# aleph-zero-foundation/sha2-on-cq-halo2

Hardware: AMD Instinct MI355X
Metric: sha256_cq_create_proof_k18: MSM Mscalar/s over proof-generation wall-clock (ms_per_step) (higher is better)
Workload: dtype u256-montgomery

## Files before the change

### sha2_on_cq_halo2_amd/csrc/curve.hpp

```cpp
#pragma once
#include "field.hpp"

namespace cq {

struct alignas(16) G1Affine {
  Fq x, y;
  CQ_HD bool is_identity() const { return x.is_zero() && y.is_zero(); }
  static CQ_HD G1Affine identity() { return {Fq::zero(), Fq::zero()}; }
  CQ_HD G1Affine neg() const { return {x, y.is_zero() ? y : y.neg()}; }
};

struct alignas(16) G1Jac {
  Fq x, y, z;
  static CQ_HD G1Jac identity() { return {Fq::zero(), Fq::zero(), Fq::zero()}; }
  CQ_HD bool is_identity() const { return z.is_zero(); }
};

struct XYZZ {
  Fq x, y, zz, zzz;
  static CQ_HD XYZZ identity() { return {Fq::zero(), Fq::zero(), Fq::zero(), Fq::zero()}; }
  CQ_HD bool is_identity() const { return zz.is_zero(); }
  static CQ_HD XYZZ from_affine(const G1Affine& a) {
    if (a.is_identity()) return identity();
    return {a.x, a.y, Fq::one(), Fq::one()};
  }
  CQ_HD G1Jac to_jac() const {
    if (is_identity()) return G1Jac::identity();
    return {x * zz, y * zzz, zz};
  }
};

static CQ_HD XYZZ xyzz_dbl_affine(const G1Affine& a) {
  if (a.is_identity() || a.y.is_zero()) return XYZZ::identity();
  Fq u = a.y.dbl();
  Fq v = u.sqr();
  Fq w = u * v;
  Fq s = a.x * v;
  Fq x2 = a.x.sqr();
  Fq m = x2.dbl() + x2;
  Fq x3 = m.sqr() - s.dbl();
  Fq y3 = m * (s - x3) - w * a.y;
  return {x3, y3, v, w};
}

static CQ_HD XYZZ xyzz_dbl(const XYZZ& p) {
  if (p.is_identity() || p.y.is_zero()) return XYZZ::identity();
  Fq u = p.y.dbl();
  Fq v = u.sqr();
  Fq w = u * v;
  Fq s = p.x * v;
  Fq x2 = p.x.sqr();
  Fq m = x2.dbl() + x2;
  Fq x3 = m.sqr() - s.dbl();
  Fq y3 = m * (s - x3) - w * p.y;
  return {x3, y3, v * p.zz, w * p.zzz};
}

static CQ_HD void xyzz_add_affine(XYZZ& acc, const G1Affine& a) {
  if (a.is_identity()) return;
  if (acc.is_identity()) {
    acc = {a.x, a.y, Fq::one(), Fq::one()};
    return;
  }
  Fq u2 = a.x * acc.zz;
  Fq s2 = a.y * acc.zzz;
  Fq p = u2 - acc.x;
  Fq r = s2 - acc.y;
  if (p.is_zero()) {
    if (r.is_zero()) {
      acc = xyzz_dbl_affine(a);
    } else {
      acc = XYZZ::identity();
    }
    return;
  }
  Fq pp = p.sqr();
  Fq ppp = p * pp;
  Fq q = acc.x * pp;
  Fq x3 = r.sqr() - ppp - q.dbl();
  Fq y3 = r * (q - x3) - acc.y * ppp;
  acc.x = x3;
  acc.y = y3;
  acc.zz = acc.zz * pp;
  acc.zzz = acc.zzz * ppp;
}

static CQ_HD void xyzz_add(XYZZ& acc, const XYZZ& b) {
  if (b.is_identity()) return;
  if (acc.is_identity()) {
    acc = b;
    return;
  }
  Fq u1 = acc.x * b.zz;
  Fq u2 = b.x * acc.zz;
  Fq s1 = acc.y * b.zzz;
  Fq s2 = b.y * acc.zzz;
  Fq p = u2 - u1;
  Fq r = s2 - s1;
  if (p.is_zero()) {
    if (r.is_zero()) {
      acc = xyzz_dbl(acc);
    } else {
      acc = XYZZ::identity();
    }
    return;
  }
  Fq pp = p.sqr();
  Fq ppp = p * pp;
  Fq q = u1 * pp;
  Fq x3 = r.sqr() - ppp - q.dbl();
  Fq y3 = r * (q - x3) - s1 * ppp;
  acc.x = x3;
  acc.y = y3;
  acc.zz = acc.zz * b.zz * pp;
  acc.zzz = acc.zzz * b.zzz * ppp;
}

static CQ_HD G1Jac jac_dbl(const G1Jac& p) {
  if (p.is_identity() || p.y.is_zero()) return G1Jac::identity();
  Fq a = p.x.sqr();
  Fq b = p.y.sqr();
  Fq c = b.sqr();
  Fq d = ((p.x + b).sqr() - a - c).dbl();
  Fq e = a.dbl() + a;
  Fq f = e.sqr();
  Fq x3 = f - d.dbl();
  Fq y3 = e * (d - x3) - c.dbl().dbl().dbl();
  Fq z3 = (p.y * p.z).dbl();
  return {x3, y3, z3};
}

static CQ_HD G1Jac jac_add(const G1Jac& p, const G1Jac& q) {
  if (p.is_identity()) return q;
  if (q.is_identity()) return p;
  Fq z1z1 = p.z.sqr();
  Fq z2z2 = q.z.sqr();
  Fq u1 = p.x * z2z2;
  Fq u2 = q.x * z1z1;
  Fq s1 = p.y * q.z * z2z2;
  Fq s2 = q.y * p.z * z1z1;
  if (u1 == u2) {
    if (s1 == s2) return jac_dbl(p);
    return G1Jac::identity();
  }
  Fq h = u2 - u1;
  Fq r = s2 - s1;
  Fq hh = h.sqr();
  Fq hhh = h * hh;
  Fq v = u1 * hh;
  Fq x3 = r.sqr() - hhh - v.dbl();
  Fq y3 = r * (v - x3) - s1 * hhh;
  Fq z3 = p.z * q.z * h;
  return {x3, y3, z3};
}

static CQ_HD G1Jac jac_from_affine(const G1Affine& a) {
  if (a.is_identity()) return G1Jac::identity();
  return {a.x, a.y, Fq::one()};
}

static CQ_HD G1Affine jac_to_affine(const G1Jac& p) {
  if (p.is_identity()) return G1Affine::identity();
  Fq zi = p.z.inv();
  Fq zi2 = zi.sqr();
  return {p.x * zi2, p.y * zi2 * zi};
}

}
```

### sha2_on_cq_halo2_amd/csrc/glv.hpp

```cpp
#pragma once
#include "curve.hpp"

namespace cq {

static const uint64_t GLV_LAMBDA_RAW[4] = {0x8b17ea66b99c90ddull, 0x5bfc41088d8daaa7ull, 0xb3c4d79d41a91758ull, 0x0ull};
static const uint64_t GLV_ZETA_RAW[4] = {0x5763473177fffffeull, 0xd4f263f1acdb5c4full, 0x59e26bcea0d48bacull, 0x0ull};
static const uint64_t GLV_G1[3] = {0xd91d232ec7e0b3d7ull, 0x2ull, 0x0ull};
static const uint64_t GLV_G2[3] = {0x7a7bd9d4391eb18dull, 0x4ccef014a773d2cfull, 0x2ull};
static const uint64_t GLV_MINUS_B1[4] = {0x8211bbeb7d4f1128ull, 0x6f4d8248eeb859fcull, 0x0ull, 0x0ull};
static const uint64_t GLV_B2[4] = {0x89d3256894d213e3ull, 0x0ull, 0x0ull, 0x0ull};

static inline void glv_mul_hi(const uint64_t* g, const uint64_t* k, uint64_t* out) {
  typedef unsigned __int128 u128;
  uint64_t prod[8] = {0, 0, 0, 0, 0, 0, 0, 0};
  for (int i = 0; i < 3; i++) {
    u128 carry = 0;
    for (int j = 0; j < 4; j++) {
      const u128 t = (u128)g[i] * k[j] + prod[i + j] + carry;
      prod[i + j] = (uint64_t)t;
      carry = t >> 64;
    }
    prod[i + 4] = (uint64_t)carry;
  }
  for (int i = 0; i < 4; i++) out[i] = i + 4 < 7 ? prod[i + 4] : 0;
}
static inline void glv_small(const Fr& v, uint64_t* mag, bool& neg) {
  static const Fr half = fr_from_raw(FR_HALF_RAW);
  uint64_t w[4];
  const U256 c = v.to_canonical();
  for (int i = 0; i < 4; i++) w[i] = (uint64_t)c.l[2 * i] | ((uint64_t)c.l[2 * i + 1] << 32);
  uint64_t hw[4];
  const U256 hc = half.to_canonical();
  for (int i = 0; i < 4; i++) hw[i] = (uint64_t)hc.l[2 * i] | ((uint64_t)hc.l[2 * i + 1] << 32);
  neg = false;
  for (int i = 3; i >= 0; i--)
    if (w[i] != hw[i]) {
      neg = w[i] > hw[i];
      break;
    }
  if (neg) {
    const U256 n = v.neg().to_canonical();
    for (int i = 0; i < 4; i++) w[i] = (uint64_t)n.l[2 * i] | ((uint64_t)n.l[2 * i + 1] << 32);
  }
  mag[0] = w[0];
  mag[1] = w[1];
}
struct GlvSplit {
  uint64_t m[2][2];
  bool neg[2];
};
inline GlvSplit glv_split(const Fr& k) {
  static const Fr lambda = fr_from_raw(GLV_LAMBDA_RAW), minus_b1 = fr_from_raw(GLV_MINUS_B1), b2 = fr_from_raw(GLV_B2);
  uint64_t kw[4], c1w[4], c2w[4];
  const U256 kc = k.to_canonical();
  for (int i = 0; i < 4; i++) kw[i] = (uint64_t)kc.l[2 * i] | ((uint64_t)kc.l[2 * i + 1] << 32);
  glv_mul_hi(GLV_G1, kw, c1w);
  glv_mul_hi(GLV_G2, kw, c2w);
  const Fr c1 = fr_from_raw(c1w), c2 = fr_from_raw(c2w);
  const Fr k2 = c1 * minus_b1 - c2 * b2;
  const Fr k1 = k - k2 * lambda;
  GlvSplit sp;
  glv_small(k1, sp.m[0], sp.neg[0]);
  glv_small(k2, sp.m[1], sp.neg[1]);
  return sp;
}
inline void glv_table(const G1Jac& p, const GlvSplit& sp, int half, G1Jac* t) {
  static const Fq zeta = Fq::from_limbs64(GLV_ZETA_RAW) * Fq::r2();
  t[0] = G1Jac::identity();
  t[1] = p;
  for (int i = 2; i < 16; i++) t[i] = (i & 1) ? jac_add(t[i - 1], p) : jac_dbl(t[i / 2]);
  for (int i = 1; i < 16; i++) {
    if (half) t[i].x = t[i].x * zeta;
    if (sp.neg[half]) t[i].y = t[i].y.neg();
  }
}
inline G1Jac host_scalar_mul_half(const G1Jac& p, const Fr& k, int half) {
  const GlvSplit sp = glv_split(k);
  G1Jac t[16];
  glv_table(p, sp, half, t);
  G1Jac acc = G1Jac::identity();
  for (int nib = 31; nib >= 0; nib--) {
    for (int d = 0; d < 4; d++) acc = jac_dbl(acc);
    const uint32_t v = (uint32_t)(sp.m[half][nib >> 4] >> ((nib & 15) * 4)) & 15u;
    if (v) acc = jac_add(acc, t[v]);
  }
  return acc;
}
inline G1Jac host_scalar_mul(const G1Jac& p, const Fr& k) {
  const GlvSplit sp = glv_split(k);
  G1Jac t1[16], t2[16];
  glv_table(p, sp, 0, t1);
  glv_table(p, sp, 1, t2);
  G1Jac acc = G1Jac::identity();
  for (int nib = 31; nib >= 0; nib--) {
    for (int d = 0; d < 4; d++) acc = jac_dbl(acc);
    const uint32_t v1 = (uint32_t)(sp.m[0][nib >> 4] >> ((nib & 15) * 4)) & 15u;
    const uint32_t v2 = (uint32_t)(sp.m[1][nib >> 4] >> ((nib & 15) * 4)) & 15u;
    if (v1) acc = jac_add(acc, t1[v1]);
    if (v2) acc = jac_add(acc, t2[v2]);
  }
  return acc;
}

}
```

### sha2_on_cq_halo2_amd/csrc/hostpool.hpp

```cpp
#pragma once
#include <atomic>
#include <condition_variable>
#include <deque>
#include <functional>
#include <memory>
#include <mutex>
#include <thread>
#include <vector>

namespace cq {

class HostPool {
 public:
  struct Job {
    std::function<void(size_t)> fn;
    size_t count = 0;
    std::atomic<size_t> next{0}, done{0};
  };
  using Ticket = std::shared_ptr<Job>;

  explicit HostPool(unsigned workers) {
    for (unsigned i = 0; i < workers; i++) {
      try {
        threads_.emplace_back([this]() { run(); });
      } catch (...) {
        break;
      }
    }
  }
  ~HostPool() {
    {
      std::lock_guard<std::mutex> lk(mu_);
      stop_ = true;
    }
    cv_.notify_all();
    for (auto& t : threads_) t.join();
  }
  HostPool(const HostPool&) = delete;
  HostPool& operator=(const HostPool&) = delete;

  Ticket submit(size_t count, std::function<void(size_t)> fn) {
    Ticket j = std::make_shared<Job>();
    j->fn = std::move(fn);
    j->count = count;
    if (count && !threads_.empty()) {
      {
        std::lock_guard<std::mutex> lk(mu_);
        queue_.push_back(j);
      }
      cv_.notify_all();
    }
    return j;
  }
  void wait(const Ticket& j) {
    if (!j) return;
    work_on(*j);
    std::unique_lock<std::mutex> lk(mu_);
    done_cv_.wait(lk, [&]() { return j->done.load() >= j->count; });
  }
  void parallel_for(size_t count, std::function<void(size_t)> fn) { wait(submit(count, std::move(fn))); }

 private:
  void work_on(Job& j) {
    for (;;) {
      const size_t i = j.next.fetch_add(1);
      if (i >= j.count) return;
      j.fn(i);
      if (j.done.fetch_add(1) + 1 == j.count) {
        std::lock_guard<std::mutex> lk(mu_);
        done_cv_.notify_all();
      }
    }
  }
  void run() {
    for (;;) {
      Ticket j;
      {
        std::unique_lock<std::mutex> lk(mu_);
        cv_.wait(lk, [&]() { return stop_ || !queue_.empty(); });
        if (stop_) return;
        j = queue_.front();
        if (j->next.load() >= j->count) {
          queue_.pop_front();
          continue;
        }
      }
      work_on(*j);
    }
  }
  std::vector<std::thread> threads_;
  std::deque<Ticket> queue_;
  std::mutex mu_;
  std::condition_variable cv_, done_cv_;
  bool stop_ = false;
};

}
```

### sha2_on_cq_halo2_amd/csrc/msm.hip

```cpp
#include <algorithm>
#include <cstdlib>
#include "msm.hpp"
#include "curve29.hpp"
#include "ctx.hpp"

namespace cq {

uint32_t msm_window_bits(uint32_t n) {
  if (n >= (1u << 15)) return 15;
  if (n >= (1u << 13)) return 10;
  if (n >= 256) return 8;
  if (n >= 16) return 4;
  return 2;
}

static_assert(msm_layout_k::XYZZ_BYTES == sizeof(XYZZ) && msm_layout_k::PTR_BYTES == sizeof(void*) && sizeof(void*) == sizeof(uint64_t),
              "the layout's byte sizes");
static_assert(sizeof(G1Affine) == 64 && sizeof(uint4) == 16, "64-byte table points; the clearing kernel stores 16 bytes");
static_assert(msm_layout_k::S1 == MSM_S1 && msm_layout_k::S1_MIN == MSM_S1_MIN && msm_layout_k::S2 == MSM_S2 &&
                  msm_layout_k::SHORT_MIN == MSM_SHORT_MIN && msm_layout_k::SMALL_LANES == MSM_SMALL_LANES &&
                  msm_layout_k::SMALL_PARTIALS == MSM_SMALL_PARTIALS && msm_layout_k::TABLE_C_MAX == MSM_TABLE_C_MAX,
              "the layout's copies of the tuning constants");

MsmBuffers::MsmBuffers(const MsmLayout& L, void* workspace) {
  char* ws = (char*)workspace;
  ptrs = (const void**)(ws + L.off_ptr_row(0));
  lists = (const void* const*)(ws + L.off_ptr_row(0));
  bases = (const G1Affine* const*)(ws + L.off_ptr_row(1));
  strides = (const uint64_t*)(ws + L.off_ptr_row(2));
  lens = (const uint64_t*)(ws + L.off_ptr_row(3));
  src = (const uint64_t*)(ws + L.off_ptr_row(4));
  counts = (uint32_t*)(ws + L.off_counts);
  cursor = (uint32_t*)(ws + L.off_cursor);
  ticket = (uint32_t*)(ws + L.off_ticket);
  zero_quads = (L.zero_end - L.off_counts) / sizeof(uint4);
  ranks = (uint32_t*)(ws + L.off_ranks);
  part_pay = (uint32_t*)(ws + L.off_part_pay());
  pay2 = L.mid ? (uint32_t*)(ws + L.off_pay2()) : nullptr;
  part_low = ws + L.off_part_low();
  low2 = L.mid ? (uint8_t*)(ws + L.off_low2()) : nullptr;
  poff = (uint32_t*)(ws + L.off_poff);
  poff2 = (uint32_t*)(ws + L.off_poff2);
  psize = (uint32_t*)(ws + L.off_psize);
  psize2 = (uint32_t*)(ws + L.off_psize2);
  totals = (uint32_t*)(ws + L.off_psize);
  index_ticket = (uint32_t*)(ws + L.off_index_ticket());
  blocksums = (uint32_t*)(ws + L.off_blocksums);
  s1_dev = (uint32_t*)(ws + L.off_s1_dev());
  off = (uint32_t*)(ws + L.off_off);
  tk = (uint32_t*)(ws + L.off_tk);
  sorted = (uint32_t*)(ws + L.off_sorted);
  buckets = (XYZZ*)(ws + L.off_buckets);
  part[0] = (XYZZ*)(ws + L.off_part[0]);
  part[1] = (XYZZ*)(ws + L.off_part[1]);
  pairs = (XYZZ*)(ws + L.off_pairs);
}

static bool alias_lists(const MsmLaunch& ln, const MsmLayout& L, MsmTableRows& rows) {
  uint32_t alias[MSM_MAX_BATCH];
  bool any_alias = false;
  for (uint32_t i = 0; i < MSM_MAX_BATCH; i++) {
    rows.lists.p[i] = i < L.batch ? ln.lists[i] : nullptr;
    rows.bases.p[i] = i < L.batch ? (const void*)ln.bases[i] : nullptr;
    rows.strides.s[i] = i < L.batch ? (uint64_t)ln.stride(i, L) : 0;
    rows.lens.s[i] = i < L.batch ? (uint64_t)ln.len(i, L) : 0;
    alias[i] = i;
    if (i < L.batch && L.part_sort)
      for (uint32_t j = 0; j < i; j++)
        if (alias[j] == j && ln.lists[j] == ln.lists[i] && ln.len(j, L) == ln.len(i, L) && ln.len(i, L)) {
          alias[i] = j;
          rows.lens.s[i] = 0;
          any_alias = true;
          break;
        }
    rows.src.s[i] = alias[i];
  }
  return any_alias;
}

static uint32_t sublist_len(const MsmLaunch& ln, const MsmLayout& L) {
  uint64_t load = 0;
  for (uint32_t i = 0; i < L.batch; i++) load = std::max<uint64_t>(load, (uint64_t)ln.len(i, L) * L.W / (L.Wb * L.M));
  const uint32_t partials = L.pre && L.Wb > 1 ? MSM_PARTIALS_TARGET / 4 : MSM_PARTIALS_TARGET;
  return load <= MSM_S1_BIG_LOAD ? msm_small_launch_s1(L.E) : std::max<uint32_t>(MSM_S1_BIG, (uint32_t)((load + partials - 1) / partials));
}

int msm_run(cq_ctx* ctx, const MsmLaunch& ln, const MsmLayout& L, void* workspace) {
  hipStream_t s = ctx->stream;
  const bool pre = L.pre, by_index = ln.by_index;
  const uint32_t n = L.n, batch = L.batch;
  if (by_index && (!L.part_sort || L.Wb != 1 || !ln.raw_out || ln.raw_count > L.B)) return -2;
  if (pre && (n > (1u << 26) || L.W > 32)) return -4;
  if (L.tmax[0] > 0xfffffff0ull || L.E > 0xfffffff0ull) return -3;
  if (batch == 0 || batch > MSM_MAX_BATCH) return -2;
  const MsmBuffers buf(L, workspace);
  MsmTableRows rows;
  const bool any_alias = alias_lists(ln, L, rows);
  const uint32_t s1 = sublist_len(ln, L);
  auto front = [&]() -> int {
    msm_enqueue_tables(s, L, buf, rows);
    if (by_index) msm_front_index(s, L, buf, s1, any_alias, ln.raw_count);
    else if (L.part_sort) msm_front_partition(s, L, buf, s1, any_alias);
    else msm_front_plain(s, L, buf, s1);
    return 0;
  };
  auto tail = [&]() -> int {
    msm_combine_levels(s, L, buf);
    if (ln.raw_out) msm_emit_buckets(s, L, buf, ln.raw_count, ln.raw_out);
    else msm_reduce_sets(s, L, buf, ln.window_sums);
    return 0;
  };
  std::vector<uint64_t> sig{(uint64_t)(uintptr_t)workspace, (uint64_t)(uintptr_t)ln.window_sums, n, L.c, batch, (pre ? 1u : 0u) | (by_index ? 2u : 0u), s1,
                            (uint64_t)(uintptr_t)ln.raw_out, ln.raw_count};
  for (uint32_t i = 0; i < batch; i++) {
    sig.push_back((uint64_t)(uintptr_t)ln.lists[i]);
    sig.push_back((uint64_t)(uintptr_t)ln.bases[i]);
    sig.push_back((uint64_t)ln.len(i, L));
    sig.push_back((uint64_t)ln.stride(i, L));
  }
  if (ctx->run_graph(sig, 0, front) != 0) return -1;
  if (ctx->prof_on && ctx->prof_entries && ctx->prof_entries_n < cq_ctx::PROF_COUNTERS)
    (void)hipMemcpyAsync(ctx->prof_entries + ctx->prof_entries_n++, buf.off + L.Bt, sizeof(uint32_t), hipMemcpyDeviceToHost, s);
  constexpr size_t TAIL_EARLY_POINTS = (size_t)1 << 20;
  const bool tail_early = n >= TAIL_EARLY_POINTS;
  const bool hand_over = ctx->msm_tail_event && !ctx->on_side_stream();
  if (tail_early && hand_over) {
    (void)hipEventRecord(ctx->msm_tail_event, s);
    ctx->msm_tail_seq++;
  }
  hipEvent_t pe = ctx->prof_begin(CQ_PROF_MSM_ACCUMULATE);
  msm_accumulate(s, L, buf);
  ctx->prof_end(pe);
  if (hand_over && !tail_early) {
    (void)hipEventRecord(ctx->msm_tail_event, s);
    ctx->msm_tail_seq++;
  }
  if (ctx->run_graph(sig, 1, tail) != 0) return -1;
  return hipGetLastError() == hipSuccess ? 0 : -1;
}

static bool bucket_sums_shape(uint32_t n, uint32_t batch) { return batch && batch <= MSM_MAX_BATCH && n && n <= (1u << 26); }
static bool bucket_sums_fit(const MsmLayout& L) { return L.E <= 0xfffffff0ull && L.tmax[0] <= 0xfffffff0ull && L.total <= ((size_t)32 << 30); }
bool msm_bucket_sums_fit(uint32_t n, uint32_t batch) { return bucket_sums_shape(n, batch) && bucket_sums_fit(MsmLayout(n, MSM_TABLE_C, batch, true)); }

int msm_bucket_sums(cq_ctx* ctx, const uint32_t* const* index, const G1Affine* const* bases29, uint32_t n, uint32_t batch, uint32_t count,
                    G1Affine* out) {
  const uint32_t c = MSM_TABLE_C;
  if (!count || count > (1u << (c - 1)) || !bucket_sums_shape(n, batch)) return -2;
  const MsmLayout L(n, c, batch, true);
  if (!bucket_sums_fit(L)) return -2;
  void* ws;
  if (ctx->ensure_scratch(ctx->on_side_stream() ? Scratch::MsmWorkAux : Scratch::MsmWork, L.total, &ws) != 0) return -1;
  const MsmLaunch ln{true, (const void* const*)index, bases29, nullptr, nullptr, nullptr, out, count};
  return msm_run(ctx, ln, L, ws);
}

G1Jac msm_set_value(const G1Jac* planes, uint32_t cols) {
  G1Jac v = planes[6];
  for (int t = 5; t >= 0; t--) v = jac_add(jac_dbl(v), planes[t]);
  if (cols == 128) {
    for (int t = 6; t >= 0; t--) v = jac_add(jac_dbl(v), planes[7 + t]);
    return jac_add(v, planes[14]);
  }
  G1Jac u = planes[13];
  for (int t = 5; t >= 0; t--) u = jac_add(jac_dbl(u), planes[7 + t]);
  for (uint32_t l = cols; l > 1; l >>= 1) v = jac_dbl(v);
  return jac_add(jac_add(v, u), planes[14]);
}

G1Jac msm_fold_sets(const G1Jac* pairs, uint32_t Wb, uint32_t M, uint32_t cols) {
  if (Wb == 1) return msm_set_value(pairs, cols);
  G1Jac planes[MSM_SET_POINTS];
  for (uint32_t q = 0; q < MSM_SET_POINTS; q++) {
    planes[q] = pairs[q];
    for (uint32_t s = 1; s < Wb; s++) planes[q] = jac_add(planes[q], pairs[(size_t)MSM_SET_POINTS * s + q]);
  }
  G1Jac acc = msm_set_value(planes, cols);
  G1Jac run = G1Jac::identity(), weighted = G1Jac::identity();
  for (uint32_t s = Wb - 1; s >= 1; s--) {
    run = jac_add(run, pairs[(size_t)MSM_SET_POINTS * s + MSM_SET_POINTS - 1]);
    weighted = jac_add(weighted, run);
  }
  for (uint32_t l = M; l > 1; l >>= 1) weighted = jac_dbl(weighted);
  return jac_add(acc, weighted);
}

G1Jac msm_fold_windows(const G1Jac* pairs, uint32_t W, uint32_t c, uint32_t cols) {
  G1Jac acc = G1Jac::identity();
  if (c >= 2 && cols == (1u << (c - 1))) {
    for (int w = (int)W - 1; w >= 0; w--) {
      const G1Jac* pl = pairs + (size_t)MSM_SET_POINTS * w;
      acc = jac_dbl(acc);
      for (int t = (int)c - 2; t >= 0; t--) acc = jac_add(jac_dbl(acc), pl[7 + t]);
      acc = jac_add(acc, pl[14]);
    }
    return acc;
  }
  for (int w = (int)W - 1; w >= 0; w--) {
    for (uint32_t j = 0; j < c; j++) acc = jac_dbl(acc);
    acc = jac_add(acc, msm_set_value(pairs + (size_t)MSM_SET_POINTS * w, cols));
  }
  return acc;
}

}
```

### sha2_on_cq_halo2_amd/csrc/msm.hpp

```cpp
#pragma once
#include <hip/hip_runtime.h>
#include <optional>
#include <vector>
#include "curve.hpp"
#include "msm_layout.hpp"

struct cq_ctx;

namespace cq {

constexpr uint32_t MSM_ACC_THREADS = 128;

#ifndef CQ_MSM_S1
#define CQ_MSM_S1 24
#endif
constexpr uint32_t MSM_S1 = CQ_MSM_S1;
#ifndef CQ_MSM_S1_BIG
#define CQ_MSM_S1_BIG 32
#endif
#ifndef CQ_MSM_S1_BIG_LOAD
#define CQ_MSM_S1_BIG_LOAD 512
#endif
constexpr uint32_t MSM_S1_BIG = CQ_MSM_S1_BIG;
constexpr uint32_t MSM_S1_BIG_LOAD = CQ_MSM_S1_BIG_LOAD;
#ifndef CQ_MSM_PARTIALS_TARGET
#define CQ_MSM_PARTIALS_TARGET 48
#endif
constexpr uint32_t MSM_PARTIALS_TARGET = CQ_MSM_PARTIALS_TARGET;
static_assert(MSM_S1_BIG >= MSM_S1, "the workspace is sized for MSM_S1");
#ifndef CQ_MSM_SMALL_LANES
#define CQ_MSM_SMALL_LANES 65536
#endif
constexpr uint32_t MSM_S1_MIN = 4;
constexpr uint64_t MSM_SMALL_LANES = CQ_MSM_SMALL_LANES;
constexpr uint64_t MSM_SMALL_PARTIALS = 3 * MSM_SMALL_LANES;
constexpr uint32_t MSM_S2 = 64;
constexpr uint32_t MSM_SHORT = 64;
constexpr uint32_t MSM_SHORT_MIN = 16;
#ifndef CQ_MSM_WAVE_BUDGET
#define CQ_MSM_WAVE_BUDGET 4096
#endif
constexpr uint32_t MSM_WAVE_BUDGET = CQ_MSM_WAVE_BUDGET;
constexpr uint32_t MSM_COMBINE_WAVE_BLOCKS = 2048;
constexpr uint32_t MSM_MAX_BATCH = 32;
constexpr uint32_t MSM_SET_POINTS = 15;

constexpr uint32_t MSM_SHORT_C = 8, MSM_SHORT_W = 32;
constexpr uint32_t MSM_SHORT_LIMIT = 1u << 14;
#ifndef CQ_MSM_SHORT_MAX
#define CQ_MSM_SHORT_MAX 16384
#endif
constexpr uint32_t MSM_SHORT_MAX = CQ_MSM_SHORT_MAX;
static_assert(MSM_SHORT_MAX <= MSM_SHORT_LIMIT && MSM_SHORT_MAX >= 4097, "the cut-over covers N + 1 = 4097 and fits the kernel");

struct MsmPtrs {
  const void* p[MSM_MAX_BATCH];
};
struct MsmStrides {
  uint64_t s[MSM_MAX_BATCH];
};

struct MsmTableRows {
  MsmPtrs lists, bases;
  MsmStrides strides, lens, src;
};

struct MsmBuffers {
  const void** ptrs;
  const void* const* lists;
  const G1Affine* const* bases;
  const uint64_t *strides, *lens, *src;
  const Fr* const* scalars() const { return (const Fr* const*)lists; }
  const uint32_t* const* index() const { return (const uint32_t* const*)lists; }
  uint32_t *counts, *cursor, *ticket;
  size_t zero_quads;
  uint32_t* ranks;
  uint32_t *part_pay, *pay2;
  void* part_low;
  uint8_t* low2;
  uint32_t *poff, *poff2;
  uint32_t *psize, *psize2;
  uint32_t *totals, *index_ticket;
  uint32_t* blocksums;
  uint32_t* s1_dev;
  uint32_t *off , *tk , *sorted;
  XYZZ *buckets, *part[2] , *pairs ;
  MsmBuffers(const MsmLayout& L, void* workspace);
};

uint32_t msm_window_bits(uint32_t n);
struct MsmLaunch {
  bool by_index;
  const void* const* lists;
  const G1Affine* const* bases;
  const size_t* lens;
  const size_t* strides;
  G1Jac* window_sums;
  G1Affine* raw_out;
  uint32_t raw_count;
  size_t len(uint32_t i, const MsmLayout& L) const { return lens ? lens[i] : L.n; }
  size_t stride(uint32_t i, const MsmLayout& L) const { return !L.pre ? 0 : strides ? strides[i] : L.n; }
};
int msm_run(cq_ctx* ctx, const MsmLaunch& ln, const MsmLayout& L, void* workspace);

void msm_enqueue_tables(hipStream_t s, const MsmLayout& L, const MsmBuffers& b, const MsmTableRows& rows);
void msm_plan(hipStream_t s, const MsmLayout& L, const MsmBuffers& b, uint32_t s1, const uint32_t* s1_dev);
void msm_front_plain(hipStream_t s, const MsmLayout& L, const MsmBuffers& b, uint32_t s1);
void msm_front_partition(hipStream_t s, const MsmLayout& L, const MsmBuffers& b, uint32_t s1, bool any_alias);
void msm_front_index(hipStream_t s, const MsmLayout& L, const MsmBuffers& b, uint32_t s1, bool any_alias, uint32_t count);
void msm_accumulate(hipStream_t s, const MsmLayout& L, const MsmBuffers& b);
void msm_combine_levels(hipStream_t s, const MsmLayout& L, const MsmBuffers& b);
void msm_reduce_sets(hipStream_t s, const MsmLayout& L, const MsmBuffers& b, G1Jac* window_sums);
void msm_emit_buckets(hipStream_t s, const MsmLayout& L, const MsmBuffers& b, uint32_t count, G1Affine* out);
size_t msm_short_workspace(uint32_t n, uint32_t batch);
int msm_short_run(cq_ctx* ctx, const Fr* const* scalars, const G1Affine* const* bases, uint32_t n, uint32_t batch, void* workspace,
                  G1Jac* window_sums_dev);
int msm_bucket_sums(cq_ctx* ctx, const uint32_t* const* index, const G1Affine* const* bases29, uint32_t n, uint32_t batch, uint32_t count,
                    G1Affine* out);
int msm_bases29(cq_ctx* ctx, const G1Affine* bases, uint32_t n, G1Affine* out);
bool msm_bucket_sums_fit(uint32_t n, uint32_t batch);
int msm_precompute_tables(cq_ctx* ctx, const G1Affine* bases, uint32_t n, uint32_t c, G1Affine* table);
G1Jac msm_set_value(const G1Jac* planes, uint32_t cols);
G1Jac msm_fold_windows(const G1Jac* pairs, uint32_t W, uint32_t c, uint32_t cols);
G1Jac msm_fold_sets(const G1Jac* pairs, uint32_t Wb, uint32_t M, uint32_t cols);

}

int cq_msm_multi(cq_ctx* c, const cq::Fr* const* scalars, const cq::G1Affine* const* bases, size_t len, size_t count,
                 uint64_t* out_jac);
int cq_msm_multi_v(cq_ctx* c, const cq::Fr* const* scalars, const cq::G1Affine* const* bases, const size_t* lens, size_t count,
                   uint64_t* out_jac);
struct MsmPending {
  struct Launch {
    size_t first = 0, slot = 0;
    uint32_t batch = 0;
    bool empty = false;
    std::optional<cq::MsmLayout> L;
    bool short_path = false;
  };
  std::vector<Launch> launches;
  void* host = nullptr;
  size_t slots = 0, count = 0;
};
int msm_multi_begin(cq_ctx* c, const cq::Fr* const* scalars, const cq::G1Affine* const* bases, const size_t* lens, size_t count,
                    MsmPending& pend);
int msm_multi_end(cq_ctx* c, MsmPending& pend, uint64_t* out_jac);
constexpr uint32_t MSM_TABLE_C = 15, MSM_TABLE_C_MIN = 8, MSM_TABLE_C_MAX = 20;
uint32_t msm_table_window_bits(size_t n);

int msm_register_tables(cq_ctx* c, const cq::G1Affine* bases, size_t n, uint32_t want_c = 0, bool* held = nullptr);
void msm_release_table(cq_ctx* c, const void* bases, size_t n, uint32_t c_bits);
void msm_unregister_tables(cq_ctx* c, const void* bases);
```

### sha2_on_cq_halo2_amd/csrc/msm_multi.hip

```cpp
#include <algorithm>
#include <cstdlib>
#include <cstring>
#include <vector>
#include "ctx.hpp"
#include "msm.hpp"

using namespace cq;

uint32_t msm_table_window_bits(size_t n) {
  if (const char* e = getenv("CQ_TABLE_C")) {
    const long v = atol(e);
    if (v >= (long)MSM_TABLE_C_MIN && v <= (long)MSM_TABLE_C_MAX) return (uint32_t)v;
  }
  return n >= ((size_t)1 << 20) ? 17u : MSM_TABLE_C;
}

static uint32_t pick_c(cq_ctx* c, uint32_t n) {
  if (c->msm_c) return c->msm_c;
  return msm_window_bits(n);
}

int msm_multi_begin(cq_ctx* c, const Fr* const* scalars, const G1Affine* const* bases, const size_t* lens, size_t count,
                    MsmPending& pend) {
  pend.launches.clear();
  pend.count = count;
  for (size_t j = 0; j < count; j++)
    if (lens[j] > 0x7fffffffull) return c->fail(CQ_ERR_ARG, "msm: len too large");
  uint32_t want_c = 0;
  {
    size_t longest = 0;
    for (size_t j = 0; j < count; j++)
      if (lens[j] > longest)
        if (const cq_ctx::MsmTable* t = c->find_msm_table(bases[j], lens[j])) { longest = lens[j]; want_c = t->c; }
  }
  size_t done = 0, slots = 0;
  while (done < count) {
    MsmPending::Launch ln;
    ln.first = done;
    if (lens[done] == 0) {
      ln.batch = 1;
      ln.empty = true;
      pend.launches.push_back(ln);
      done++;
      continue;
    }
    const cq_ctx::MsmTable* t0 = c->find_msm_table(bases[done], lens[done], nullptr, want_c);
    const bool pre = t0 != nullptr;
    uint32_t nmax = (uint32_t)lens[done];
    uint32_t batch = 1;
    while (done + batch < count && batch < MSM_MAX_BATCH) {
      const size_t l = lens[done + batch];
      if (l == 0) break;
      const cq_ctx::MsmTable* t = c->find_msm_table(bases[done + batch], l, nullptr, want_c);
      if ((t != nullptr) != pre) break;
      if (pre && t->c != t0->c) break;
      if (!pre && l != lens[done]) break;
      nmax = std::max(nmax, (uint32_t)l);
      batch++;
    }
    ln.short_path = !pre && !c->msm_c && nmax <= MSM_SHORT_MAX;
    const uint32_t cb = pre ? t0->c : ln.short_path ? MSM_SHORT_C : pick_c(c, nmax);
    ln.L.emplace(nmax, cb, batch, pre);
    while (batch > 1 && ln.L->total > ((size_t)32 << 30)) {
      batch = (batch + 1) / 2;
      ln.L.emplace(nmax, cb, batch, pre);
    }
    ln.batch = batch;
    ln.slot = slots;
    slots += (size_t)MSM_SET_POINTS * batch * ln.L->Wb;
    pend.launches.push_back(ln);
    done += batch;
  }
  void *wsums = nullptr, *host = nullptr;
  int rc;
  if (slots) {
    if ((rc = c->ensure_scratch(Scratch::MsmSums, slots * sizeof(G1Jac), &wsums)) != CQ_OK) return rc;
    if ((rc = c->ensure_pinned_msm(slots * sizeof(G1Jac), &host)) != CQ_OK) return rc;
  }
  pend.host = host;
  pend.slots = slots;
  for (auto& ln : pend.launches) {
    if (ln.empty) continue;
    const MsmLayout& L = *ln.L;
    if (ln.short_path) {
      void* ws;
      if ((rc = c->ensure_scratch(Scratch::MsmWork, msm_short_workspace(L.n, ln.batch), &ws)) != CQ_OK) return rc;
      if (msm_short_run(c, scalars + ln.first, bases + ln.first, L.n, ln.batch, ws, (G1Jac*)wsums + ln.slot) != 0)
        return c->fail(CQ_ERR_HIP, "msm launch failed");
      continue;
    }
    std::vector<const G1Affine*> bp(ln.batch);
    std::vector<size_t> strides(ln.batch, 0);
    for (uint32_t j = 0; j < ln.batch; j++) {
      size_t toff = 0;
      const cq_ctx::MsmTable* t = L.pre ? c->find_msm_table(bases[ln.first + j], lens[ln.first + j], &toff, L.c) : nullptr;
      bp[j] = L.pre ? (const G1Affine*)t->table + toff : bases[ln.first + j];
      strides[j] = L.pre ? t->n : 0;
    }
    void* ws;
    if ((rc = c->ensure_scratch(Scratch::MsmWork, L.total, &ws)) != CQ_OK) return rc;
    const MsmLaunch run{false, (const void* const*)(scalars + ln.first), bp.data(),
                        lens + ln.first, strides.data(), (G1Jac*)wsums + ln.slot, nullptr, 0};
    if (msm_run(c, run, L, ws) != 0) return c->fail(CQ_ERR_HIP, "msm launch failed");
  }
  if (slots)
    CQ_HIP(c, hipMemcpyAsync(host, wsums, slots * sizeof(G1Jac), hipMemcpyDeviceToHost, c->stream));
  return CQ_OK;
}

int msm_multi_end(cq_ctx* c, MsmPending& pend, uint64_t* out_jac) {
  if (int wrc = c->wait(c->stream, "msm: waiting for the launch")) return wrc;
  struct Item { const MsmPending::Launch* ln; uint32_t j; };
  std::vector<Item> items;
  size_t sets = 0;
  for (auto& ln : pend.launches)
    for (uint32_t j = 0; j < ln.batch; j++) {
      items.push_back({&ln, j});
      if (!ln.empty) sets += ln.L->Wb;
    }
  const G1Jac* host = (const G1Jac*)pend.host;
  auto fold = [&](size_t i) {
    const MsmPending::Launch& ln = *items[i].ln;
    const uint32_t j = items[i].j;
    uint64_t* o = out_jac + (ln.first + j) * 12;
    if (ln.empty) {
      memset(o, 0, 12 * sizeof(uint64_t));
      return;
    }
    const G1Jac* res = host + ln.slot;
    const MsmLayout& L = *ln.L;
    G1Jac r = L.pre ? msm_fold_sets(res + (size_t)MSM_SET_POINTS * j * L.Wb, L.Wb, L.M, L.cols)
                    : msm_fold_windows(res + (size_t)MSM_SET_POINTS * j * L.W, L.W, L.c, L.cols);
    r.x.to_limbs64(o);
    r.y.to_limbs64(o + 4);
    r.z.to_limbs64(o + 8);
  };
  if (sets > 6) {
    c->pool().parallel_for(items.size(), fold);
  } else {
    for (size_t i = 0; i < items.size(); i++) fold(i);
  }
  return CQ_OK;
}

int cq_msm_multi_v(cq_ctx* c, const Fr* const* scalars, const G1Affine* const* bases, const size_t* lens, size_t count,
                   uint64_t* out_jac) {
  MsmPending pend;
  int rc = msm_multi_begin(c, scalars, bases, lens, count, pend);
  if (rc != CQ_OK) return rc;
  return msm_multi_end(c, pend, out_jac);
}

int cq_msm_multi(cq_ctx* c, const Fr* const* scalars, const G1Affine* const* bases, size_t len, size_t count,
                 uint64_t* out_jac) {
  std::vector<size_t> lens(count, len);
  return cq_msm_multi_v(c, scalars, bases, lens.data(), count, out_jac);
}

void msm_unregister_tables(cq_ctx* c, const void* bases) {
  for (size_t i = 0; i < c->msm_tables.size();) {
    if (c->msm_tables[i].bases == bases) {
      hipFree(c->msm_tables[i].table);
      c->msm_tables.erase(c->msm_tables.begin() + i);
    } else {
      i++;
    }
  }
}

void msm_release_table(cq_ctx* c, const void* bases, size_t n, uint32_t c_bits) {
  for (size_t i = 0; i < c->msm_tables.size(); i++) {
    cq_ctx::MsmTable& t = c->msm_tables[i];
    if (t.bases != bases || t.n != n || t.c != c_bits) continue;
    if (--t.refs == 0) {
      hipFree(t.table);
      c->msm_tables.erase(c->msm_tables.begin() + i);
    }
    return;
  }
}

int msm_register_tables(cq_ctx* c, const G1Affine* bases, size_t n, uint32_t want_c, bool* held) {
  if (held) *held = false;
  if (!bases || n == 0 || n > (1u << 26)) return CQ_OK;
  const uint32_t cb = want_c ? want_c : (c->msm_table_c ? c->msm_table_c : msm_table_window_bits(n));
  for (auto& t : c->msm_tables)
    if (t.bases == bases && t.n == n && t.c == cb) {
      t.refs++;
      if (held) *held = true;
      return CQ_OK;
    }
  {
    size_t off = 0;
    const cq_ctx::MsmTable* t = c->find_msm_table(bases, n, &off, cb);
    if (t && (t->c == cb || !want_c)) return CQ_OK;
  }
  const uint32_t W = (255 + cb - 1) / cb;
  void* table = nullptr;
  if (hipMalloc(&table, (size_t)W * n * sizeof(G1Affine)) != hipSuccess) {
    (void)hipGetLastError();
    return CQ_OK;
  }
  if (msm_precompute_tables(c, bases, (uint32_t)n, cb, (G1Affine*)table) != 0) {
    hipFree(table);
    return c->fail(CQ_ERR_HIP, "msm precompute failed");
  }
  c->msm_tables.push_back({bases, n, cb, table, 1});
  if (held) *held = true;
  return CQ_OK;
}
```

### sha2_on_cq_halo2_amd/csrc/prover_lookup.hip

```cpp
#include "prover_run.hpp"

namespace cq {
namespace prover {

GateEvalArgs ProofRun::lagrange_eval_args(const uint32_t* prog, uint32_t num_polys, const Fr& fold) const {
  GateEvalArgs ga;
  ga.prog = prog;
  ga.num_polys = num_polys;
  ga.constants = pk->constants;
  ga.challenges = B.challenges;
  ga.advice = B.adv;
  ga.fixed = pk->fixed_values;
  ga.instance = B.inst_lag;
  ga.stride = n;
  ga.size = (uint32_t)n;
  ga.rot_scale = 1;
  ga.y = fold;
  return ga;
}
int ProofRun::lagrange_compress(const uint32_t* prog, uint32_t width, const Fr& chal, Fr* dst) {
  return gate_eval(c, lagrange_eval_args(prog, width, chal), dst);
}

int ProofRun::count_multiplicities() {
  if (!L) return CQ_OK;
  CQ_HIP(c, hipMemsetAsync(B.m_counts, 0, (L * N + 16) * sizeof(uint32_t), s));
  size_t input_slot = 0;
  CqRound1Batch r1b;
  r1b.count = 0;
  for (size_t l = 0; l < L; l++) {
    const cq_lookup_desc& lk = pk->lookups[l];
    const uint32_t w = (uint32_t)lk.cols.size();
    for (uint32_t j = 0; j < w; j++, input_slot++) {
      if (lk.prog[j] < 0) {
        lk_input[l][j] = B.adv + (size_t)lk.cols[j] * n;
        continue;
      }
      Fr* dst = B.lk_inputs + input_slot * n;
      CQ_TRY(gate_eval(c, lagrange_eval_args(pk->lookup_prog + lk.prog[j], 1, Fr::zero()), dst));
      lk_input[l][j] = dst;
    }
    CqRound1Args& ra = r1b.a[r1b.count];
    ra.width = w;
    for (uint32_t j = 0; j < w; j++) {
      ra.cols[j] = lk_input[l][j];
      ra.values[j] = lk.tables[j]->values;
      ra.slots[j] = lk.tables[j]->slots;
      ra.nslots[j] = lk.tables[j]->nslots;
    }
    r1b.bucket[r1b.count] = b_by_rows ? B.b_index + l * n : nullptr;
    r1b.n = b_by_rows ? (uint32_t)n : 0;
    r1b.blind_bucket = (uint32_t)N;
    r1b.m_counts[r1b.count++] = B.m_counts + l * N;
    if (r1b.count == CQ_ROUND1_BATCH || l + 1 == L) {
      CQ_TRY(cq::cq_round1(c, r1b, u, B.err_dev));
      r1b.count = 0;
    }
  }
  CQ_TRY(cq_m_to_fr(c, B.m_counts, (uint32_t)(L * N), B.m_fr));
  if (!sums_side) CQ_TRY(bucket_sum_launches());
  *herr = 0;
  CQ_HIP(c, hipMemcpyAsync((void*)herr, B.err_dev, 4, hipMemcpyDeviceToHost, s));
  return CQ_OK;
}
int ProofRun::bucket_sum_launches() {
  for (size_t l0 = 0; b_by_rows && l0 < L; l0 += MSM_MAX_BATCH / 2) {
    std::vector<const uint32_t*> sc;
    std::vector<const G1Affine*> bs;
    for (size_t l = l0; l < std::min(L, l0 + MSM_MAX_BATCH / 2); l++)
      for (int q = 0; q < 2; q++) { sc.push_back(B.b_index + l * n); bs.push_back(pk->b_row_bases[q]); }
    if (msm_bucket_sums(c, sc.data(), bs.data(), (uint32_t)n, (uint32_t)sc.size(), (uint32_t)(N + 1), B.b_sums + 2 * l0 * (N + 1)) != 0)
      return c->fail(CQ_ERR_HIP, "bucket-sum launch failed");
  }
  return CQ_OK;
}
int ProofRun::lookup_error() {
  if (*herr == 1) return c->fail(CQ_ERR_LOOKUP, "witness value not in table");
  if (*herr == 2) return c->fail(CQ_ERR_LOOKUP, "Vector lookup must be on the same table row");
  return CQ_OK;
}

int ProofRun::legacy_commit_permuted() {
  if (!PL) return CQ_OK;
  void* stage_v;
  const size_t slot = n * 4;
  CQ_TRY(c->ensure_scratch(Scratch::ProverStage, 3 * slot * sizeof(uint64_t) + lookup_permute_scratch_bytes(k) + 64, &stage_v));
  uint64_t* stage = (uint64_t*)stage_v;
  void* lk_scratch = stage + 3 * slot;
  uint32_t* lk_status = (uint32_t*)((char*)lk_scratch + lookup_permute_scratch_bytes(k));
  uint32_t* lk_status_host = (uint32_t*)((char*)small_v + 16);
  for (size_t l = 0; l < PL; l++) {
    const auto& lk = pk->legacy[l];
    CQ_TRY(lagrange_compress(pk->legacy_prog + lk.in_off, lk.width, theta, plk_buf(l, 0)));
    CQ_TRY(lagrange_compress(pk->legacy_prog + lk.tab_off, lk.width, theta, plk_buf(l, 1)));
    CQ_TRY(fr_to_canonical(c, plk_buf(l, 0), u, stage));
    CQ_TRY(fr_to_canonical(c, plk_buf(l, 1), u, stage + slot));
    CQ_TRY(lookup_permute_dev(c, stage, stage + slot, u, k, stage + 2 * slot, lk_scratch, lk_status));
    CQ_HIP(c, hipMemcpyAsync(lk_status_host, lk_status, 3 * sizeof(uint32_t), hipMemcpyDeviceToHost, s));
    CQ_TRY(fr_from_canonical(c, stage, u, plk_buf(l, 2)));
    CQ_TRY(fr_from_canonical(c, stage + 2 * slot, u, plk_buf(l, 3)));
    CQ_HIP(c, hipMemcpyAsync(plk_buf(l, 2) + u, plk_tails.data() + l * 2 * (bf + 1), (bf + 1) * sizeof(Fr), hipMemcpyHostToDevice, s));
    CQ_HIP(c, hipMemcpyAsync(plk_buf(l, 3) + u, plk_tails.data() + l * 2 * (bf + 1) + (bf + 1), (bf + 1) * sizeof(Fr), hipMemcpyHostToDevice, s));
    CQ_TRY(c->wait(s));
    if (lk_status_host[0] != 0 || lk_status_host[1] != lk_status_host[2])
      return c->fail(CQ_ERR_LOOKUP, "lookup input not in table (Error::ConstraintSystemFailure)");
  }
  return CQ_OK;
}

int ProofRun::cq_round1() {
  if (L && !early_m) {
    CQ_TRY(count_multiplicities());
    CQ_TRY(c->wait(s));
    CQ_TRY(lookup_error());
  }
  theta_pow[0] = Fr::one();
  for (uint32_t j = 1; j < CQ_MAX_WIDTH; j++) theta_pow[j] = theta_pow[j - 1] * theta;
  for (size_t l0 = 0; l0 < L; l0 += CQ_FOLD_BATCH) {
    CqFoldBatch fb;
    fb.count = (uint32_t)std::min<size_t>(CQ_FOLD_BATCH, L - l0);
    for (uint32_t j = 0; j < CQ_MAX_WIDTH; j++) fb.theta_pow[j] = theta_pow[j];
    for (uint32_t q = 0; q < fb.count; q++) {
      const size_t l = l0 + q;
      const uint32_t w = (uint32_t)pk->lookups[l].cols.size();
      fb.width[q] = w;
      for (uint32_t j = 0; j < w; j++) fb.src[q][j] = lk_input[l][j];
      fb.out[q] = owns_lookup(l) ? B.f_lag + l * n : nullptr;
    }
    CQ_TRY(cq_fold_inputs(c, fb, (uint32_t)n));
  }
  if (L || PL) {
    std::vector<const Fr*> sc;
    std::vector<const G1Affine*> bs;
    std::vector<size_t> ln;
    for (size_t l = 0; l < PL; l++)
      for (int which = 2; which <= 3; which++) { sc.push_back(plk_buf(l, which)); bs.push_back(pk->params->g_lagrange); ln.push_back(n); }
    std::vector<int> f_linear(L, 0);
    std::vector<G1Jac> f_host(L);
    for (size_t l = 0; l < L; l++) {
      f_linear[l] = 1;
      for (int64_t pj : pk->lookups[l].prog) f_linear[l] &= pj < 0;
    }
    std::vector<size_t> f_slot(L, 0);
    for (size_t l = 0; l < L; l++)
      if (!f_linear[l]) { f_slot[l] = sc.size(); sc.push_back(B.f_lag + l * n); bs.push_back(pk->params->g_lagrange); ln.push_back(n); }
    const size_t m_first = sc.size();
    if (!early_m)
      for (size_t l = 0; l < L; l++) { sc.push_back(B.m_fr + l * N); bs.push_back(pk->table_cfg->g1_lagrange); ln.push_back(N); }
    std::vector<G1Affine> cm;
    Commit r1;
    const uint64_t seq = c->msm_tail_seq;
    if (!sc.empty()) CQ_TRY(r1.begin(pk, sc, bs, ln));
    if (L && !early_m) CQ_TRY(fork_bucket_sums(seq));
    std::vector<size_t> f_lin;
    for (size_t l = 0; l < L; l++)
      if (f_linear[l]) f_lin.push_back(l);
    struct PoolJoin {
      HostPool& pool;
      HostPool::Ticket t;
      ~PoolJoin() { pool.wait(t); }
    } f_job{c->pool(), nullptr};
    f_job.t = c->pool().submit(f_lin.size(), [&](size_t i) {
      const size_t l = f_lin[i];
      const auto& lcols = pk->lookups[l].cols;
      G1Jac acc = jac_from_affine(advice_commitments[lcols[0]]);
      for (size_t j = 1; j < lcols.size(); j++) acc = jac_add(host_scalar_mul(acc, theta), jac_from_affine(advice_commitments[lcols[j]]));
      f_host[l] = acc;
    });
    {
      AuxFork fork(c);
      CQ_TRY(fork.begin(seq));
      if (resident) {
        CQ_TRY(resident_round1_transforms());
      } else {
        if (L) {
          CQ_TRY(lagrange_to_coeff_cols(B.f_lag, B.f_coeff, L));
          CQ_TRY(coeff_to_extended_cols(B.f_coeff, B.cosets + L * ext, L));
        }
        if (general && I) CQ_TRY(coeff_to_extended_cols(B.inst_coeff, B.inst_cosets, I));
        if (A && S == 0 && !adv_is_coeff) {
          CQ_TRY(lagrange_to_coeff_cols(B.adv, B.adv, A));
          adv_is_coeff = true;
        }
      }
      CQ_TRY(fork.end());
    }
    if (!sc.empty()) CQ_TRY(r1.end(cm));
    c->pool().wait(f_job.t);
    for (size_t q = 0; q < 2 * PL; q++)
      if (!tr.write_point(cm[q])) return c->fail(CQ_ERR_TRANSCRIPT, "permuted lookup commitment is the identity");
    for (size_t l = 0; l < L; l++) {
      const G1Affine f_cm = f_linear[l] ? jac_to_affine(f_host[l]) : cm[f_slot[l]];
      if (!tr.write_point(f_cm)) return c->fail(CQ_ERR_TRANSCRIPT, "f commitment is the identity");
      if (!tr.write_point(early_m ? m_commitments[l] : cm[m_first + l])) return c->fail(CQ_ERR_TRANSCRIPT, "m commitment is the identity");
    }
  }
  return CQ_OK;
}

int ProofRun::legacy_commit_product() {
  for (size_t l = 0; l < PL; l++)
    CQ_TRY(lookup_product(c, plk_buf(l, 0), plk_buf(l, 1), plk_buf(l, 2), plk_buf(l, 3), beta, gamma, plkz_tails.data() + l * bf, (uint32_t)n, bf,
                          plk_buf(l, 4)));
  return CQ_OK;
}

int ProofRun::cq_round2() {
  bool random_late = false;
  CQ_TRY(round2_prepare());
  CQ_TRY(round2_random_late(random_late));
  return round2_commit(random_late);
}
int ProofRun::round2_prepare() {
  for (size_t l0 = 0; l0 < L; l0 += CQ_FOLD_BATCH) {
    CqFoldBatch fb;
    fb.count = (uint32_t)std::min<size_t>(CQ_FOLD_BATCH, L - l0);
    for (uint32_t j = 0; j < CQ_MAX_WIDTH; j++) fb.theta_pow[j] = theta_pow[j];
    for (uint32_t q = 0; q < fb.count; q++) {
      const size_t l = l0 + q;
      const cq_lookup_desc& lk = pk->lookups[l];
      fb.width[q] = (uint32_t)lk.cols.size();
      for (uint32_t j = 0; j < fb.width[q]; j++) fb.src[q][j] = lk.tables[j]->values;
      fb.out[q] = nullptr;
      fb.f[q] = owns_lookup(l) ? B.f_lag + l * n : nullptr;
      fb.b[q] = B.bpoly + l * n;
      fb.m[q] = B.m_counts + l * N;
      fb.den[q] = B.den + l * N;
    }
    CQ_TRY(cq_round2_prep(c, fb, (uint32_t)n, (uint32_t)N, u, beta));
  }
  if (resident) {
    CQ_TRY(resident_round2_invert());
  } else if (L) {
    CQ_TRY(poly_batch_invert(c, B.bpoly, (uint32_t)(L * n + L * N)));
  }
  size_t woff = 0;
  for (size_t l0 = 0; l0 < L; l0 += CQ_FOLD_BATCH) {
    CqAValuesBatch ab;
    ab.count = (uint32_t)std::min<size_t>(CQ_FOLD_BATCH, L - l0);
    ab.beta_inv = beta_inv;
    for (uint32_t j = 0; j < CQ_MAX_WIDTH; j++) ab.theta_pow[j] = theta_pow[j];
    for (uint32_t q = 0; q < ab.count; q++) {
      const size_t l = l0 + q;
      ab.width[q] = (uint32_t)pk->lookups[l].cols.size();
      ab.den_inv[q] = B.den + l * N;
      ab.m[q] = B.m_counts + l * N;
      ab.a[q] = B.a_val + l * N;
      ab.a_scaled[q] = B.a_scaled + woff * N;
      ab.b_values[q] = b_by_rows ? B.b_values + l * (N + 1) : nullptr;
      woff += ab.width[q];
    }
    CQ_TRY(cq_a_values_batch(c, ab, (uint32_t)N));
  }
  if (resident) {
    CQ_TRY(resident_round2_b_to_coeff());
  } else if (L) {
    CQ_TRY(lagrange_to_coeff_cols(B.bpoly, B.bpoly, L));
    GatherArgs ga;
    ga.count = (uint32_t)L;
    for (size_t l = 0; l < L; l++) ga.src[l] = B.bpoly + l * n;
    CQ_TRY(poly_gather_scalars(c, ga, B.gather));
    CQ_HIP(c, hipMemcpyAsync(small_fr, B.gather, L * sizeof(Fr), hipMemcpyDeviceToHost, s));
  }
  return CQ_OK;
}
int ProofRun::round2_random_late(bool& random_late) {
  const char* force = getenv("CQ_RANDOM_LATE");
  const auto t0 = std::chrono::steady_clock::now();
  while (!drawer.done.load()) {
    if (force && force[0] == '1') break;
    const double waited = std::chrono::duration<double, std::micro>(std::chrono::steady_clock::now() - t0).count();
    if (!(force && force[0] == '0') && waited > 100.0 && drawer.remaining_us() > 700.0) break;
    std::this_thread::yield();
  }
  CQ_TRY(shard_any(pk, (force && force[0] == '1') || !drawer.done.load(), random_late));
  return CQ_OK;
}
int ProofRun::round2_commit(bool random_late) {
  if (!random_late) CQ_TRY(finish_random_poly());
  std::vector<G1Affine> r2;
  {
    std::vector<const Fr*> sc;
    std::vector<const G1Affine*> bs;
    std::vector<size_t> ln;
    std::vector<size_t> at;
    for (size_t l = 0; b_by_rows && l < L; l++)
      for (size_t q = 0; q < 2; q++) { sc.push_back(B.b_values + l * (N + 1)); bs.push_back(B.b_sums + (2 * l + q) * (N + 1)); ln.push_back(N + 1); }
    for (size_t st = 0; st < S; st++) { at.push_back(sc.size()); sc.push_back(B.z + st * n); bs.push_back(pk->params->g_lagrange); ln.push_back(n); }
    for (size_t l = 0; l < PL; l++) { at.push_back(sc.size()); sc.push_back(plk_buf(l, 4)); bs.push_back(pk->params->g_lagrange); ln.push_back(n); }
    size_t woff = 0;
    for (size_t l = 0; l < L; l++) {
      const uint32_t w = (uint32_t)pk->lookups[l].cols.size();
      at.push_back(sc.size()); sc.push_back(B.a_val + l * N); bs.push_back(pk->table_cfg->g1_lagrange); ln.push_back(N);
      at.push_back(sc.size()); sc.push_back(B.a_scaled + woff * N); bs.push_back(pk->qs_concat[l]); ln.push_back((size_t)w * N);
      at.push_back(sc.size()); sc.push_back(B.a_val + l * N); bs.push_back(pk->table_cfg->g_lagrange_opening_at_0); ln.push_back(N);
      if (b_by_rows) {
        at.push_back(2 * l);
        at.push_back(2 * l + 1);
      } else {
        at.push_back(sc.size()); sc.push_back(B.bpoly + l * n + 1); bs.push_back(pk->params->g); ln.push_back(n - 1);
        at.push_back(sc.size()); sc.push_back(B.bpoly + l * n + 1); bs.push_back(pk->b0_g1_bound); ln.push_back(n - 1);
      }
      woff += w;
    }
    if (!random_late) { at.push_back(sc.size()); sc.push_back(B.random_poly); bs.push_back(pk->params->g); ln.push_back(n); }
    Commit r2cm;
    const uint64_t seq = c->msm_tail_seq;
    if (sums_pending) {
      CQ_HIP(c, hipStreamWaitEvent(s, c->b_sums_done, 0));
      sums_pending = false;
    }
    CQ_TRY(r2cm.begin(pk, sc, bs, ln));
    {
      AuxFork fork(c);
      CQ_TRY(fork.begin(seq));
      if (A && !adv_is_coeff) CQ_TRY(lagrange_to_coeff_cols(B.adv, B.adv, A));
      if (resident) CQ_TRY(resident_b_to_coset());
      else if (L) CQ_TRY(coeff_to_extended_cols(B.bpoly, B.cosets, L));
      if (general && A) CQ_TRY(coeff_to_extended_cols(B.adv, B.adv_cosets, A));
      CQ_TRY(fork.end());
    }
    if (random_late) CQ_TRY(finish_random_poly());
    mark("round 2 queued");
    {
      std::vector<G1Affine> in_launch_order;
      CQ_TRY(r2cm.end(in_launch_order));
      for (size_t i : at) r2.push_back(in_launch_order[i]);
    }
    mark("round 2 commitments on the host");
    if (random_late) {
      std::vector<G1Affine> rc;
      CQ_TRY(commit_batch(pk, {B.random_poly}, {pk->params->g}, n, rc));
      r2.push_back(rc[0]);
    }
  }
  for (size_t st = 0; st < S; st++)
    if (!tr.write_point(r2[st])) return c->fail(CQ_ERR_TRANSCRIPT, "permutation product commitment is the identity");
  if (S) CQ_TRY(lagrange_to_coeff_cols(B.z, B.z, S));
  for (size_t l = 0; l < PL; l++) {
    if (!tr.write_point(r2[S + l])) return c->fail(CQ_ERR_TRANSCRIPT, "lookup product commitment is the identity");
    CQ_TRY(domain_lagrange_to_coeff(dom, plk_buf(l, 2), plk_buf(l, 2), 3, n, n));
  }
  for (size_t l = 0; l < L; l++) {
    for (size_t q = 0; q < 5; q++)
      if (!tr.write_point(r2[S + PL + 5 * l + q])) return c->fail(CQ_ERR_TRANSCRIPT, "a CQ round-2 commitment is the identity");
  }
  random_cm = r2[S + PL + 5 * L];
  if (L) {
    if (resident) CQ_TRY(resident_sum_b_at_zero());
    const Fr n_table_inv = Fr::from_u64(N).inv();
    for (size_t l = 0; l < L; l++)
      a_at_zero[l] = (small_fr[l] * Fr::from_u64(n) - Fr::from_u64(bf + 1) * beta_inv) * n_table_inv;
  }
  return CQ_OK;
}

}
}
```

### sha2_on_cq_halo2_amd/csrc/prover_support.hip

```cpp
#include "prover_run.hpp"

namespace cq {
namespace prover {

namespace {

void batch_normalize(const std::vector<G1Jac>& in, std::vector<G1Affine>& out) {
  out.resize(in.size());
  std::vector<Fq> pref(in.size());
  Fq acc = Fq::one();
  for (size_t i = 0; i < in.size(); i++) {
    pref[i] = acc;
    if (!in[i].is_identity()) acc = acc * in[i].z;
  }
  acc = acc.inv();
  for (size_t i = in.size(); i-- > 0;) {
    if (in[i].is_identity()) {
      out[i] = G1Affine::identity();
      continue;
    }
    Fq zi = pref[i] * acc;
    acc = acc * in[i].z;
    Fq zi2 = zi.sqr();
    out[i] = {in[i].x * zi2, in[i].y * zi2 * zi};
  }
}

G1Jac jac_from_limbs(const uint64_t* l) {
  return {Fq::from_limbs64(l), Fq::from_limbs64(l + 4), Fq::from_limbs64(l + 8)};
}

}

bool host_trace_enabled() {
  static const bool on = getenv("CQ_TRACE_HOST") != nullptr;
  return on;
}

void Rng::fill(uint64_t* dst, size_t count) {
  if (bulk) {
    bulk(state, dst, count);
  } else if (next == cq_xoshiro256ss_next_u64) {
    xoshiro_fill((uint64_t*)state, dst, count, 8, pool);
  } else if (next == cq_buffer_rng_next_u64) {
    cq_buffer_rng* b = (cq_buffer_rng*)state;
    const size_t avail = b->pos < b->len ? b->len - b->pos : 0, take = std::min(avail, count);
    memcpy(dst, b->words + b->pos, take * sizeof(uint64_t));
    memset(dst + take, 0, (count - take) * sizeof(uint64_t));
    b->pos += take;
    b->overrun += count - take;
  } else {
    for (size_t i = 0; i < count; i++) dst[i] = next(state);
  }
}

int Commit::begin(const cq_pk* pk_, const std::vector<const Fr*>& scalars, const std::vector<const G1Affine*>& bases,
                  const std::vector<size_t>& lens) {
  pk = pk_;
  count = scalars.size();
  if (!pk->sharded()) return msm_multi_begin(pk->ctx, scalars.data(), bases.data(), lens.data(), count, pend);
  std::vector<const Fr*> sc(count);
  std::vector<const G1Affine*> bs(count);
  std::vector<size_t> ln(count);
  for (size_t j = 0; j < count; j++) {
    size_t lo, hi;
    shard_range(lens[j], pk->shard_rank, pk->shard_world, lo, hi);
    sc[j] = scalars[j] + lo;
    bs[j] = bases[j] + lo;
    ln[j] = hi - lo;
  }
  return msm_multi_begin(pk->ctx, sc.data(), bs.data(), ln.data(), count, pend);
}
int Commit::end(std::vector<G1Affine>& out) {
  cq_ctx* c = pk->ctx;
  std::vector<uint64_t> jac(count * 12);
  const bool trace_host = host_trace_enabled();
  const auto t0 = std::chrono::steady_clock::now();
  if (trace_host) hipStreamSynchronize(c->stream);
  const auto t1 = std::chrono::steady_clock::now();
  int rc = msm_multi_end(c, pend, jac.data());
  if (rc != CQ_OK) return rc;
  const auto t2 = std::chrono::steady_clock::now();
  struct Report {
    bool on; std::chrono::steady_clock::time_point a, b, c_;
    ~Report() {
      if (on) fprintf(stderr, "[cq host]   commit end: wait %.1f us, fold %.1f us, exchange + normalise %.1f us\n",
                      std::chrono::duration<double, std::micro>(b - a).count(), std::chrono::duration<double, std::micro>(c_ - b).count(),
                      std::chrono::duration<double, std::micro>(std::chrono::steady_clock::now() - c_).count());
    }
  } report{trace_host, t0, t1, t2};
  std::vector<G1Jac> j(count);
  if (pk->sharded()) {
    std::vector<uint64_t> all((size_t)pk->shard_world * count * 12);
    int arc = shard_allgather_host(pk, jac.data(), all.data(), count * 12 * sizeof(uint64_t));
    if (arc != CQ_OK) return arc;
    for (size_t i = 0; i < count; i++) {
      G1Jac acc = G1Jac::identity();
      for (uint32_t r = 0; r < pk->shard_world; r++) acc = jac_add(acc, jac_from_limbs(all.data() + ((size_t)r * count + i) * 12));
      j[i] = acc;
    }
  } else {
    for (size_t i = 0; i < count; i++) j[i] = jac_from_limbs(jac.data() + 12 * i);
  }
  batch_normalize(j, out);
  return CQ_OK;
}

int shard_any(const cq_pk* pk, bool flag, bool& out) {
  out = flag;
  if (!pk->sharded()) return CQ_OK;
  const uint64_t mine = flag ? 1 : 0;
  std::vector<uint64_t> all(pk->shard_world, 0);
  int arc = shard_allgather_host(pk, &mine, all.data(), sizeof(uint64_t));
  if (arc != CQ_OK) return arc;
  for (uint64_t v : all) out = out || v != 0;
  return CQ_OK;
}

int commit_batch_v(const cq_pk* pk, const std::vector<const Fr*>& scalars, const std::vector<const G1Affine*>& bases,
                   const std::vector<size_t>& lens, std::vector<G1Affine>& out) {
  Commit cm;
  int rc = cm.begin(pk, scalars, bases, lens);
  if (rc != CQ_OK) return rc;
  return cm.end(out);
}

int commit_batch(const cq_pk* pk, const std::vector<const Fr*>& scalars, const std::vector<const G1Affine*>& bases, size_t len,
                 std::vector<G1Affine>& out) {
  std::vector<size_t> lens(scalars.size(), len);
  return commit_batch_v(pk, scalars, bases, lens, out);
}

bool early_advice_polys(const cq_pk* pk) {
  return !pk->general() && pk->perm_sets() == 0 && pk->num_phases == 1 && pk->num_advice > 0 && !pk->lookups.empty();
}

void carve(const cq_pk* pk, Arena& ar, Buffers& b) {
  const size_t n = (size_t)1 << pk->k, ext = pk->domain->ext();
  const size_t L = pk->lookups.size(), A = pk->num_advice, I = pk->num_instance, S = pk->perm_sets();
  const size_t N = pk->table_cfg ? pk->table_cfg->N : 0;
  const bool general = pk->general();
  size_t wsum = 0;
  for (auto& lk : pk->lookups) wsum += lk.cols.size();
  const size_t npts = pk->opening_rotations().size();
  b.adv = ar.take(A * n);
  b.adv_coeff = ar.take(early_advice_polys(pk) ? A * n : 0);
  b.inst_lag = ar.take(I * n);
  b.inst_coeff = ar.take(I * n);
  b.f_lag = ar.take(L * n);
  b.f_coeff = ar.take(L * n);
  b.bpoly = ar.take(L * n);
  b.den = ar.take(L * N + 8);
  b.random_poly = ar.take(n);
  b.z = ar.take(S * n);
  b.mv = ar.take(S * n);
  b.cosets = ar.take(2 * L * ext);
  b.adv_cosets = ar.take(general ? A * ext : 0);
  b.inst_cosets = ar.take(general ? I * ext : 0);
  b.z_cosets = ar.take(S * ext);
  b.lk_inputs = ar.take(pk->lookup_exprs ? wsum * n : 0);
  b.plk = ar.take(pk->legacy.size() * 5 * n);
  b.plk_cosets = ar.take(pk->legacy.size() * 5 * ext);
  b.h_ext = ar.take(ext);
  b.h_coeff = ar.take(ext);
  const bool shplonk = pk->opener == CQ_OPENER_SHPLONK;
  b.gwc_batch = ar.take(shplonk ? 0 : npts * n);
  b.gwc_wit = ar.take(shplonk ? 0 : npts * n);
  b.shplonk = ar.take(shplonk ? 5 * n + 64 * 8 : 0);
  b.a_val = ar.take(L * N);
  b.m_fr = ar.take(L * N);
  b.a_scaled = ar.take(wsum * N);
  b.b_values = ar.take(pk->b_row_bases[0] ? (L * (N + 1) + 1) & ~(size_t)1 : 0);
  b.b_sums = (G1Affine*)ar.take(pk->b_row_bases[0] ? 2 * 2 * L * (N + 1) : 0);
  b.b_index = (uint32_t*)ar.take(pk->b_row_bases[0] ? (L * n + 7) / 8 : 0);
  b.challenges = ar.take(pk->challenge_phase.size() + 8);
  b.tails = ar.take(A * (pk->bf + 1) + 8);
  b.gather = ar.take(GATHER_MAX);
  b.rng_dev = (uint64_t*)ar.take(2 * n);
  b.m_counts = (uint32_t*)ar.take(L * N / 8 + 64);
  b.err_dev = b.m_counts ? b.m_counts + L * N : nullptr;
}

int lincomb_many(cq_ctx* c, const std::vector<Term>& terms, const Fr& sub_const, uint32_t n, Fr* out) {
  size_t done = 0;
  bool first = true;
  do {
    LincombArgs la;
    la.count = 0;
    la.sub_const = Fr::zero();
    if (!first) {
      la.p[0] = out;
      la.len[0] = n;
      la.coeff[0] = Fr::one();
      la.count = 1;
    }
    while (done < terms.size() && la.count < LINCOMB_MAX) {
      la.p[la.count] = terms[done].p;
      la.len[la.count] = terms[done].len;
      la.coeff[la.count] = terms[done].coeff;
      la.count++;
      done++;
    }
    if (done == terms.size()) la.sub_const = sub_const;
    int rc = poly_lincomb(c, la, n, out);
    if (rc != CQ_OK) return rc;
    first = false;
  } while (done < terms.size());
  return CQ_OK;
}

int eval_many(cq_ctx* c, const std::vector<const Fr*>& ps, const std::vector<uint32_t>& ls, const Fr& z, Fr* out) {
  for (size_t off = 0; off < ps.size(); off += EVAL_MAX_BATCH) {
    const uint32_t cnt = (uint32_t)std::min((size_t)EVAL_MAX_BATCH, ps.size() - off);
    int rc = poly_eval_batch(c, ps.data() + off, ls.data() + off, cnt, z, out + off);
    if (rc != CQ_OK) return rc;
  }
  return CQ_OK;
}

void RandomPolyDrawer::start(cq_ctx* c, Rng* rng, uint64_t* pin, uint64_t* dev, size_t words) {
  const size_t chunk = std::max<size_t>(words / 4, (size_t)1 << 18);
  chunks_total = (uint32_t)((words + chunk - 1) / chunk);
  t_start = std::chrono::steady_clock::now();
  auto work = [=]() {
    hipError_t e = hipSetDevice(c->device);
    for (size_t off = 0; off < words && e == hipSuccess; off += chunk) {
      const size_t cnt = std::min(chunk, words - off);
      rng->fill(pin + off, cnt);
      e = hipMemcpyAsync(dev + off, pin + off, cnt * sizeof(uint64_t), hipMemcpyHostToDevice, c->copy_stream);
      chunks_done.fetch_add(1);
    }
    (void)rng->fr();
    if (e == hipSuccess) e = hipEventRecord(c->copy_done, c->copy_stream);
    err = e;
    done.store(true);
  };
  try {
    th = std::thread(work);
    running = true;
  } catch (...) {
    work();
  }
}
int RandomPolyDrawer::join() {
  if (running) {
    th.join();
    running = false;
  }
  return err == hipSuccess ? 0 : -1;
}

}
}
```

Baseline: 1426.

## Use 64-bit host field arithmetic for MSM folding and split long window folds

Adds a host-only 64-bit-limb Montgomery field type built on 128-bit multiplies and templates the Jacobian curve ops over it. Host-side MSM bucket folding, GLV scalar multiplication, batch normalisation and lookup f-commitment combination now use it instead of the 32-bit-limb device field type. Long window folds are also split into two halves run on separate pool threads and joined with an atomic counter, and a mixed Jacobian-affine add replaces a full add in the lookup path. These target host-side serial fold latency after the GPU MSM returns, at the cost of conversions between the two representations and extra code.

After: 1442, median of 6. +1.1%, better.

```diff
diff --git a/sha2_on_cq_halo2_amd/csrc/curve.hpp b/sha2_on_cq_halo2_amd/csrc/curve.hpp
--- a/sha2_on_cq_halo2_amd/csrc/curve.hpp
+++ b/sha2_on_cq_halo2_amd/csrc/curve.hpp
@@ -1,5 +1,6 @@
 #pragma once
 #include "field.hpp"
+#include "hostfield.hpp"
 
 namespace cq {
 
@@ -116,41 +117,68 @@
   acc.zzz = acc.zzz * b.zzz * ppp;
 }
 
-static CQ_HD G1Jac jac_dbl(const G1Jac& p) {
-  if (p.is_identity() || p.y.is_zero()) return G1Jac::identity();
-  Fq a = p.x.sqr();
-  Fq b = p.y.sqr();
-  Fq c = b.sqr();
-  Fq d = ((p.x + b).sqr() - a - c).dbl();
-  Fq e = a.dbl() + a;
-  Fq f = e.sqr();
-  Fq x3 = f - d.dbl();
-  Fq y3 = e * (d - x3) - c.dbl().dbl().dbl();
-  Fq z3 = (p.y * p.z).dbl();
+template <class J>
+static CQ_HD J jac_dbl(const J& p) {
+  typedef decltype(J::x) F;
+  if (p.is_identity() || p.y.is_zero()) return J::identity();
+  F a = p.x.sqr();
+  F b = p.y.sqr();
+  F c = b.sqr();
+  F d = ((p.x + b).sqr() - a - c).dbl();
+  F e = a.dbl() + a;
+  F f = e.sqr();
+  F x3 = f - d.dbl();
+  F y3 = e * (d - x3) - c.dbl().dbl().dbl();
+  F z3 = (p.y * p.z).dbl();
   return {x3, y3, z3};
 }
 
-static CQ_HD G1Jac jac_add(const G1Jac& p, const G1Jac& q) {
+template <class J>
+static CQ_HD J jac_add(const J& p, const J& q) {
+  typedef decltype(J::x) F;
   if (p.is_identity()) return q;
   if (q.is_identity()) return p;
-  Fq z1z1 = p.z.sqr();
-  Fq z2z2 = q.z.sqr();
-  Fq u1 = p.x * z2z2;
-  Fq u2 = q.x * z1z1;
-  Fq s1 = p.y * q.z * z2z2;
-  Fq s2 = q.y * p.z * z1z1;
+  F z1z1 = p.z.sqr();
+  F z2z2 = q.z.sqr();
+  F u1 = p.x * z2z2;
+  F u2 = q.x * z1z1;
+  F s1 = p.y * q.z * z2z2;
+  F s2 = q.y * p.z * z1z1;
   if (u1 == u2) {
     if (s1 == s2) return jac_dbl(p);
-    return G1Jac::identity();
-  }
-  Fq h = u2 - u1;
-  Fq r = s2 - s1;
-  Fq hh = h.sqr();
-  Fq hhh = h * hh;
-  Fq v = u1 * hh;
-  Fq x3 = r.sqr() - hhh - v.dbl();
-  Fq y3 = r * (v - x3) - s1 * hhh;
-  Fq z3 = p.z * q.z * h;
+    return J::identity();
+  }
+  F h = u2 - u1;
+  F r = s2 - s1;
+  F hh = h.sqr();
+  F hhh = h * hh;
+  F v = u1 * hh;
+  F x3 = r.sqr() - hhh - v.dbl();
+  F y3 = r * (v - x3) - s1 * hhh;
+  F z3 = p.z * q.z * h;
+  return {x3, y3, z3};
+}
+
+template <class J, class A>
+static CQ_HD J jac_add_mixed(const J& p, const A& q) {
+  typedef decltype(J::x) F;
+  if (q.is_identity()) return p;
+  if (p.is_identity()) return {q.x, q.y, F::one()};
+  F z1z1 = p.z.sqr();
+  F u2 = q.x * z1z1;
+  F s2 = q.y * p.z * z1z1;
+  if (p.x == u2) {
+    if (p.y == s2) return jac_dbl(p);
+    return J::identity();
+  }
+  F h = u2 - p.x;
+  F r = s2 - p.y;
+  F hh = h.sqr();
+  F hhh = h * hh;
+  F v = p.x * hh;
+  F x3 = r.sqr() - hhh - v.dbl();
+  F y3 = r * (v - x3) - p.y * hhh;
+  F z3 = p.z * h;
   return {x3, y3, z3};
 }
 
@@ -166,4 +194,38 @@
   return {p.x * zi2, p.y * zi2 * zi};
 }
 
-}
+struct HAffine {
+  HFq x, y;
+  bool is_identity() const { return x.is_zero() && y.is_zero(); }
+  static HAffine from(const G1Affine& a) { return {HFq::from_fp(a.x), HFq::from_fp(a.y)}; }
+  G1Affine to() const { return {x.to_fp(), y.to_fp()}; }
+};
+
+struct HJac {
+  HFq x, y, z;
+  static HJac identity() { return {HFq::zero(), HFq::zero(), HFq::zero()}; }
+  bool is_identity() const { return z.is_zero(); }
+  static HJac from(const G1Jac& p) { return {HFq::from_fp(p.x), HFq::from_fp(p.y), HFq::from_fp(p.z)}; }
+  static HJac from_affine(const G1Affine& a) { return a.is_identity() ? identity() : HJac{HFq::from_fp(a.x), HFq::from_fp(a.y), HFq::one()}; }
+  G1Jac to() const { return {x.to_fp(), y.to_fp(), z.to_fp()}; }
+  static HJac from_limbs64(const uint64_t* l) { return {HFq::from_limbs64(l), HFq::from_limbs64(l + 4), HFq::from_limbs64(l + 8)}; }
+  void to_limbs64(uint64_t* l) const {
+    x.to_limbs64(l);
+    y.to_limbs64(l + 4);
+    z.to_limbs64(l + 8);
+  }
+};
+
+inline G1Jac jac_load(const G1Jac& p, const G1Jac*) { return p; }
+inline HJac jac_load(const G1Jac& p, const HJac*) { return HJac::from(p); }
+inline G1Jac jac_store(const G1Jac& p) { return p; }
+inline G1Jac jac_store(const HJac& p) { return p.to(); }
+
+inline HAffine jac_to_affine(const HJac& p) {
+  if (p.is_identity()) return {HFq::zero(), HFq::zero()};
+  HFq zi = p.z.inv();
+  HFq zi2 = zi.sqr();
+  return {p.x * zi2, p.y * zi2 * zi};
+}
+
+}
diff --git a/sha2_on_cq_halo2_amd/csrc/glv.hpp b/sha2_on_cq_halo2_amd/csrc/glv.hpp
--- a/sha2_on_cq_halo2_amd/csrc/glv.hpp
+++ b/sha2_on_cq_halo2_amd/csrc/glv.hpp
@@ -24,24 +24,16 @@
   }
   for (int i = 0; i < 4; i++) out[i] = i + 4 < 7 ? prod[i + 4] : 0;
 }
-static inline void glv_small(const Fr& v, uint64_t* mag, bool& neg) {
-  static const Fr half = fr_from_raw(FR_HALF_RAW);
+static inline void glv_small(const HFr& v, uint64_t* mag, bool& neg) {
   uint64_t w[4];
-  const U256 c = v.to_canonical();
-  for (int i = 0; i < 4; i++) w[i] = (uint64_t)c.l[2 * i] | ((uint64_t)c.l[2 * i + 1] << 32);
-  uint64_t hw[4];
-  const U256 hc = half.to_canonical();
-  for (int i = 0; i < 4; i++) hw[i] = (uint64_t)hc.l[2 * i] | ((uint64_t)hc.l[2 * i + 1] << 32);
+  v.to_canonical(w);
   neg = false;
   for (int i = 3; i >= 0; i--)
-    if (w[i] != hw[i]) {
-      neg = w[i] > hw[i];
+    if (w[i] != FR_HALF_RAW[i]) {
+      neg = w[i] > FR_HALF_RAW[i];
       break;
     }
-  if (neg) {
-    const U256 n = v.neg().to_canonical();
-    for (int i = 0; i < 4; i++) w[i] = (uint64_t)n.l[2 * i] | ((uint64_t)n.l[2 * i + 1] << 32);
-  }
+  if (neg) v.neg().to_canonical(w);
   mag[0] = w[0];
   mag[1] = w[1];
 }
@@ -49,24 +41,24 @@
   uint64_t m[2][2];
   bool neg[2];
 };
-inline GlvSplit glv_split(const Fr& k) {
-  static const Fr lambda = fr_from_raw(GLV_LAMBDA_RAW), minus_b1 = fr_from_raw(GLV_MINUS_B1), b2 = fr_from_raw(GLV_B2);
+inline GlvSplit glv_split(const Fr& k_) {
+  static const HFr lambda = HFr::from_raw(GLV_LAMBDA_RAW), minus_b1 = HFr::from_raw(GLV_MINUS_B1), b2 = HFr::from_raw(GLV_B2);
+  const HFr k = HFr::from_fp(k_);
   uint64_t kw[4], c1w[4], c2w[4];
-  const U256 kc = k.to_canonical();
-  for (int i = 0; i < 4; i++) kw[i] = (uint64_t)kc.l[2 * i] | ((uint64_t)kc.l[2 * i + 1] << 32);
+  k.to_canonical(kw);
   glv_mul_hi(GLV_G1, kw, c1w);
   glv_mul_hi(GLV_G2, kw, c2w);
-  const Fr c1 = fr_from_raw(c1w), c2 = fr_from_raw(c2w);
-  const Fr k2 = c1 * minus_b1 - c2 * b2;
-  const Fr k1 = k - k2 * lambda;
+  const HFr c1 = HFr::from_raw(c1w), c2 = HFr::from_raw(c2w);
+  const HFr k2 = c1 * minus_b1 - c2 * b2;
+  const HFr k1 = k - k2 * lambda;
   GlvSplit sp;
   glv_small(k1, sp.m[0], sp.neg[0]);
   glv_small(k2, sp.m[1], sp.neg[1]);
   return sp;
 }
-inline void glv_table(const G1Jac& p, const GlvSplit& sp, int half, G1Jac* t) {
-  static const Fq zeta = Fq::from_limbs64(GLV_ZETA_RAW) * Fq::r2();
-  t[0] = G1Jac::identity();
+inline void glv_table(const HJac& p, const GlvSplit& sp, int half, HJac* t) {
+  static const HFq zeta = HFq::from_raw(GLV_ZETA_RAW);
+  t[0] = HJac::identity();
   t[1] = p;
   for (int i = 2; i < 16; i++) t[i] = (i & 1) ? jac_add(t[i - 1], p) : jac_dbl(t[i / 2]);
   for (int i = 1; i < 16; i++) {
@@ -74,11 +66,11 @@
     if (sp.neg[half]) t[i].y = t[i].y.neg();
   }
 }
-inline G1Jac host_scalar_mul_half(const G1Jac& p, const Fr& k, int half) {
+inline HJac host_scalar_mul_half(const HJac& p, const Fr& k, int half) {
   const GlvSplit sp = glv_split(k);
-  G1Jac t[16];
+  HJac t[16];
   glv_table(p, sp, half, t);
-  G1Jac acc = G1Jac::identity();
+  HJac acc = HJac::identity();
   for (int nib = 31; nib >= 0; nib--) {
     for (int d = 0; d < 4; d++) acc = jac_dbl(acc);
     const uint32_t v = (uint32_t)(sp.m[half][nib >> 4] >> ((nib & 15) * 4)) & 15u;
@@ -86,12 +78,12 @@
   }
   return acc;
 }
-inline G1Jac host_scalar_mul(const G1Jac& p, const Fr& k) {
+inline HJac host_scalar_mul(const HJac& p, const Fr& k) {
   const GlvSplit sp = glv_split(k);
-  G1Jac t1[16], t2[16];
+  HJac t1[16], t2[16];
   glv_table(p, sp, 0, t1);
   glv_table(p, sp, 1, t2);
-  G1Jac acc = G1Jac::identity();
+  HJac acc = HJac::identity();
   for (int nib = 31; nib >= 0; nib--) {
     for (int d = 0; d < 4; d++) acc = jac_dbl(acc);
     const uint32_t v1 = (uint32_t)(sp.m[0][nib >> 4] >> ((nib & 15) * 4)) & 15u;
@@ -101,5 +93,7 @@
   }
   return acc;
 }
+inline G1Jac host_scalar_mul_half(const G1Jac& p, const Fr& k, int half) { return host_scalar_mul_half(HJac::from(p), k, half).to(); }
+inline G1Jac host_scalar_mul(const G1Jac& p, const Fr& k) { return host_scalar_mul(HJac::from(p), k).to(); }
 
 }
diff --git a/sha2_on_cq_halo2_amd/csrc/hostfield.hpp b/sha2_on_cq_halo2_amd/csrc/hostfield.hpp
--- /dev/null
+++ b/sha2_on_cq_halo2_amd/csrc/hostfield.hpp
@@ -0,0 +1,196 @@
+#pragma once
+#include "field.hpp"
+
+namespace cq {
+
+template <class P>
+struct HostFp {
+  typedef unsigned __int128 u128;
+  uint64_t l[4];
+
+  static constexpr uint64_t limb64(const uint32_t* w, int i) { return (uint64_t)w[2 * i] | ((uint64_t)w[2 * i + 1] << 32); }
+  static constexpr uint64_t M0 = limb64(P::MOD, 0), M1 = limb64(P::MOD, 1), M2 = limb64(P::MOD, 2), M3 = limb64(P::MOD, 3);
+  static constexpr uint64_t INV = (uint64_t)P::INV * (2 + M0 * (uint64_t)P::INV);
+  static_assert((uint64_t)(M0 * INV) == ~(uint64_t)0, "INV is -p^-1 mod 2^64");
+  static_assert(M3 < ((uint64_t)1 << 62), "p < 2^254: sums of two residues and the reduction's result fit four limbs");
+
+  static HostFp zero() { return {{0, 0, 0, 0}}; }
+  static HostFp one() { return {{limb64(P::R, 0), limb64(P::R, 1), limb64(P::R, 2), limb64(P::R, 3)}}; }
+  static HostFp r2() { return {{limb64(P::R2, 0), limb64(P::R2, 1), limb64(P::R2, 2), limb64(P::R2, 3)}}; }
+  static HostFp from_fp(const Fp<P>& a) {
+    HostFp r;
+    a.to_limbs64(r.l);
+    return r;
+  }
+  Fp<P> to_fp() const { return Fp<P>::from_limbs64(l); }
+  static HostFp from_limbs64(const uint64_t* s) { return {{s[0], s[1], s[2], s[3]}}; }
+  void to_limbs64(uint64_t* d) const {
+    d[0] = l[0];
+    d[1] = l[1];
+    d[2] = l[2];
+    d[3] = l[3];
+  }
+
+  bool is_zero() const { return (l[0] | l[1] | l[2] | l[3]) == 0; }
+  bool operator==(const HostFp& b) const { return ((l[0] ^ b.l[0]) | (l[1] ^ b.l[1]) | (l[2] ^ b.l[2]) | (l[3] ^ b.l[3])) == 0; }
+  bool operator!=(const HostFp& b) const { return !(*this == b); }
+
+  static uint64_t mac(uint64_t a, uint64_t b, uint64_t c, uint64_t& carry) {
+    const u128 t = (u128)b * c + a + carry;
+    carry = (uint64_t)(t >> 64);
+    return (uint64_t)t;
+  }
+  static uint64_t adc(uint64_t a, uint64_t b, uint64_t& carry) {
+    const u128 t = (u128)a + b + carry;
+    carry = (uint64_t)(t >> 64);
+    return (uint64_t)t;
+  }
+  static uint64_t sbb(uint64_t a, uint64_t b, uint64_t& borrow) {
+    const u128 t = (u128)a - b - borrow;
+    borrow = (uint64_t)(t >> 64) & 1;
+    return (uint64_t)t;
+  }
+
+  static HostFp reduce_once(uint64_t r0, uint64_t r1, uint64_t r2, uint64_t r3) {
+    uint64_t br = 0;
+    const uint64_t t0 = sbb(r0, M0, br), t1 = sbb(r1, M1, br), t2 = sbb(r2, M2, br), t3 = sbb(r3, M3, br);
+    return br ? HostFp{{r0, r1, r2, r3}} : HostFp{{t0, t1, t2, t3}};
+  }
+
+  HostFp operator+(const HostFp& b) const {
+    uint64_t c = 0;
+    const uint64_t r0 = adc(l[0], b.l[0], c), r1 = adc(l[1], b.l[1], c), r2 = adc(l[2], b.l[2], c), r3 = adc(l[3], b.l[3], c);
+    return reduce_once(r0, r1, r2, r3);
+  }
+  HostFp operator-(const HostFp& b) const {
+    uint64_t br = 0;
+    const uint64_t r0 = sbb(l[0], b.l[0], br), r1 = sbb(l[1], b.l[1], br), r2 = sbb(l[2], b.l[2], br), r3 = sbb(l[3], b.l[3], br);
+    const uint64_t mask = (uint64_t)0 - br;
+    uint64_t c = 0;
+    HostFp r;
+    r.l[0] = adc(r0, M0 & mask, c);
+    r.l[1] = adc(r1, M1 & mask, c);
+    r.l[2] = adc(r2, M2 & mask, c);
+    r.l[3] = adc(r3, M3 & mask, c);
+    return r;
+  }
+  HostFp neg() const { return zero() - *this; }
+  HostFp dbl() const {
+    const uint64_t r0 = l[0] << 1, r1 = (l[1] << 1) | (l[0] >> 63), r2 = (l[2] << 1) | (l[1] >> 63), r3 = (l[3] << 1) | (l[2] >> 63);
+    return reduce_once(r0, r1, r2, r3);
+  }
+
+  static HostFp montgomery_reduce(uint64_t r0, uint64_t r1, uint64_t r2, uint64_t r3, uint64_t r4, uint64_t r5, uint64_t r6, uint64_t r7) {
+    uint64_t carry = 0, carry2 = 0;
+    uint64_t k = r0 * INV;
+    (void)mac(r0, k, M0, carry);
+    r1 = mac(r1, k, M1, carry);
+    r2 = mac(r2, k, M2, carry);
+    r3 = mac(r3, k, M3, carry);
+    r4 = adc(r4, carry, carry2);
+
+    k = r1 * INV;
+    carry = 0;
+    (void)mac(r1, k, M0, carry);
+    r2 = mac(r2, k, M1, carry);
+    r3 = mac(r3, k, M2, carry);
+    r4 = mac(r4, k, M3, carry);
+    r5 = adc(r5, carry, carry2);
+
+    k = r2 * INV;
+    carry = 0;
+    (void)mac(r2, k, M0, carry);
+    r3 = mac(r3, k, M1, carry);
+    r4 = mac(r4, k, M2, carry);
+    r5 = mac(r5, k, M3, carry);
+    r6 = adc(r6, carry, carry2);
+
+    k = r3 * INV;
+    carry = 0;
+    (void)mac(r3, k, M0, carry);
+    r4 = mac(r4, k, M1, carry);
+    r5 = mac(r5, k, M2, carry);
+    r6 = mac(r6, k, M3, carry);
+    r7 = adc(r7, carry, carry2);
+    return reduce_once(r4, r5, r6, r7);
+  }
+
+  HostFp operator*(const HostFp& b) const {
+    uint64_t carry = 0;
+    const uint64_t r0 = mac(0, l[0], b.l[0], carry);
+    uint64_t r1 = mac(0, l[0], b.l[1], carry);
+    uint64_t r2 = mac(0, l[0], b.l[2], carry);
+    uint64_t r3 = mac(0, l[0], b.l[3], carry);
+    uint64_t r4 = carry;
+    carry = 0;
+    r1 = mac(r1, l[1], b.l[0], carry);
+    r2 = mac(r2, l[1], b.l[1], carry);
+    r3 = mac(r3, l[1], b.l[2], carry);
+    r4 = mac(r4, l[1], b.l[3], carry);
+    uint64_t r5 = carry;
+    carry = 0;
+    r2 = mac(r2, l[2], b.l[0], carry);
+    r3 = mac(r3, l[2], b.l[1], carry);
+    r4 = mac(r4, l[2], b.l[2], carry);
+    r5 = mac(r5, l[2], b.l[3], carry);
+    uint64_t r6 = carry;
+    carry = 0;
+    r3 = mac(r3, l[3], b.l[0], carry);
+    r4 = mac(r4, l[3], b.l[1], carry);
+    r5 = mac(r5, l[3], b.l[2], carry);
+    r6 = mac(r6, l[3], b.l[3], carry);
+    const uint64_t r7 = carry;
+    return montgomery_reduce(r0, r1, r2, r3, r4, r5, r6, r7);
+  }
+
+  HostFp sqr() const {
+    uint64_t carry = 0;
+    uint64_t r1 = mac(0, l[0], l[1], carry);
+    uint64_t r2 = mac(0, l[0], l[2], carry);
+    uint64_t r3 = mac(0, l[0], l[3], carry);
+    uint64_t r4 = carry;
+    carry = 0;
+    r3 = mac(r3, l[1], l[2], carry);
+    r4 = mac(r4, l[1], l[3], carry);
+    uint64_t r5 = carry;
+    carry = 0;
+    r5 = mac(r5, l[2], l[3], carry);
+    uint64_t r6 = carry;
+
+    uint64_t r7 = r6 >> 63;
+    r6 = (r6 << 1) | (r5 >> 63);
+    r5 = (r5 << 1) | (r4 >> 63);
+    r4 = (r4 << 1) | (r3 >> 63);
+    r3 = (r3 << 1) | (r2 >> 63);
+    r2 = (r2 << 1) | (r1 >> 63);
+    r1 = r1 << 1;
+
+    carry = 0;
+    uint64_t c2 = 0;
+    const uint64_t r0 = mac(0, l[0], l[0], carry);
+    r1 = adc(r1, carry, c2);
+    carry = c2;
+    c2 = 0;
+    r2 = mac(r2, l[1], l[1], carry);
+    r3 = adc(r3, carry, c2);
+    carry = c2;
+    c2 = 0;
+    r4 = mac(r4, l[2], l[2], carry);
+    r5 = adc(r5, carry, c2);
+    carry = c2;
+    c2 = 0;
+    r6 = mac(r6, l[3], l[3], carry);
+    r7 = adc(r7, carry, c2);
+    return montgomery_reduce(r0, r1, r2, r3, r4, r5, r6, r7);
+  }
+
+  void to_canonical(uint64_t* out) const { montgomery_reduce(l[0], l[1], l[2], l[3], 0, 0, 0, 0).to_limbs64(out); }
+  static HostFp from_raw(const uint64_t* raw) { return from_limbs64(raw) * r2(); }
+
+  HostFp inv() const { return from_fp(to_fp().inv()); }
+};
+
+using HFr = HostFp<FrP>;
+using HFq = HostFp<FqP>;
+
+}
diff --git a/sha2_on_cq_halo2_amd/csrc/hostpool.hpp b/sha2_on_cq_halo2_amd/csrc/hostpool.hpp
--- a/sha2_on_cq_halo2_amd/csrc/hostpool.hpp
+++ b/sha2_on_cq_halo2_amd/csrc/hostpool.hpp
@@ -59,6 +59,7 @@
     done_cv_.wait(lk, [&]() { return j->done.load() >= j->count; });
   }
   void parallel_for(size_t count, std::function<void(size_t)> fn) { wait(submit(count, std::move(fn))); }
+  size_t workers() const { return threads_.size(); }
 
  private:
   void work_on(Job& j) {
diff --git a/sha2_on_cq_halo2_amd/csrc/msm.hip b/sha2_on_cq_halo2_amd/csrc/msm.hip
--- a/sha2_on_cq_halo2_amd/csrc/msm.hip
+++ b/sha2_on_cq_halo2_amd/csrc/msm.hip
@@ -155,52 +155,8 @@
   return msm_run(ctx, ln, L, ws);
 }
 
-G1Jac msm_set_value(const G1Jac* planes, uint32_t cols) {
-  G1Jac v = planes[6];
-  for (int t = 5; t >= 0; t--) v = jac_add(jac_dbl(v), planes[t]);
-  if (cols == 128) {
-    for (int t = 6; t >= 0; t--) v = jac_add(jac_dbl(v), planes[7 + t]);
-    return jac_add(v, planes[14]);
-  }
-  G1Jac u = planes[13];
-  for (int t = 5; t >= 0; t--) u = jac_add(jac_dbl(u), planes[7 + t]);
-  for (uint32_t l = cols; l > 1; l >>= 1) v = jac_dbl(v);
-  return jac_add(jac_add(v, u), planes[14]);
-}
-
-G1Jac msm_fold_sets(const G1Jac* pairs, uint32_t Wb, uint32_t M, uint32_t cols) {
-  if (Wb == 1) return msm_set_value(pairs, cols);
-  G1Jac planes[MSM_SET_POINTS];
-  for (uint32_t q = 0; q < MSM_SET_POINTS; q++) {
-    planes[q] = pairs[q];
-    for (uint32_t s = 1; s < Wb; s++) planes[q] = jac_add(planes[q], pairs[(size_t)MSM_SET_POINTS * s + q]);
-  }
-  G1Jac acc = msm_set_value(planes, cols);
-  G1Jac run = G1Jac::identity(), weighted = G1Jac::identity();
-  for (uint32_t s = Wb - 1; s >= 1; s--) {
-    run = jac_add(run, pairs[(size_t)MSM_SET_POINTS * s + MSM_SET_POINTS - 1]);
-    weighted = jac_add(weighted, run);
-  }
-  for (uint32_t l = M; l > 1; l >>= 1) weighted = jac_dbl(weighted);
-  return jac_add(acc, weighted);
-}
-
-G1Jac msm_fold_windows(const G1Jac* pairs, uint32_t W, uint32_t c, uint32_t cols) {
-  G1Jac acc = G1Jac::identity();
-  if (c >= 2 && cols == (1u << (c - 1))) {
-    for (int w = (int)W - 1; w >= 0; w--) {
-      const G1Jac* pl = pairs + (size_t)MSM_SET_POINTS * w;
-      acc = jac_dbl(acc);
-      for (int t = (int)c - 2; t >= 0; t--) acc = jac_add(jac_dbl(acc), pl[7 + t]);
-      acc = jac_add(acc, pl[14]);
-    }
-    return acc;
-  }
-  for (int w = (int)W - 1; w >= 0; w--) {
-    for (uint32_t j = 0; j < c; j++) acc = jac_dbl(acc);
-    acc = jac_add(acc, msm_set_value(pairs + (size_t)MSM_SET_POINTS * w, cols));
-  }
-  return acc;
-}
+G1Jac msm_set_value(const G1Jac* planes, uint32_t cols) { return msm_set_value_of_t<HJac>(planes, cols).to(); }
+G1Jac msm_fold_sets(const G1Jac* pairs, uint32_t Wb, uint32_t M, uint32_t cols) { return msm_fold_sets_t<HJac>(pairs, Wb, M, cols).to(); }
+G1Jac msm_fold_windows(const G1Jac* pairs, uint32_t W, uint32_t c, uint32_t cols) { return msm_fold_windows_t<HJac>(pairs, W, c, cols).to(); }
 
 }
diff --git a/sha2_on_cq_halo2_amd/csrc/msm.hpp b/sha2_on_cq_halo2_amd/csrc/msm.hpp
--- a/sha2_on_cq_halo2_amd/csrc/msm.hpp
+++ b/sha2_on_cq_halo2_amd/csrc/msm.hpp
@@ -3,6 +3,7 @@
 #include <optional>
 #include <vector>
 #include "curve.hpp"
+#include "msm_fold.hpp"
 #include "msm_layout.hpp"
 
 struct cq_ctx;
@@ -43,7 +44,6 @@
 constexpr uint32_t MSM_WAVE_BUDGET = CQ_MSM_WAVE_BUDGET;
 constexpr uint32_t MSM_COMBINE_WAVE_BLOCKS = 2048;
 constexpr uint32_t MSM_MAX_BATCH = 32;
-constexpr uint32_t MSM_SET_POINTS = 15;
 
 constexpr uint32_t MSM_SHORT_C = 8, MSM_SHORT_W = 32;
 constexpr uint32_t MSM_SHORT_LIMIT = 1u << 14;
@@ -144,7 +144,7 @@
 };
 int msm_multi_begin(cq_ctx* c, const cq::Fr* const* scalars, const cq::G1Affine* const* bases, const size_t* lens, size_t count,
                     MsmPending& pend);
-int msm_multi_end(cq_ctx* c, MsmPending& pend, uint64_t* out_jac);
+int msm_multi_end(cq_ctx* c, MsmPending& pend, uint64_t* out_jac, bool split_long = false);
 constexpr uint32_t MSM_TABLE_C = 15, MSM_TABLE_C_MIN = 8, MSM_TABLE_C_MAX = 20;
 uint32_t msm_table_window_bits(size_t n);
 
diff --git a/sha2_on_cq_halo2_amd/csrc/msm_fold.hpp b/sha2_on_cq_halo2_amd/csrc/msm_fold.hpp
--- /dev/null
+++ b/sha2_on_cq_halo2_amd/csrc/msm_fold.hpp
@@ -0,0 +1,88 @@
+#pragma once
+#include "curve.hpp"
+
+namespace cq {
+
+constexpr uint32_t MSM_SET_POINTS = 15;
+
+template <class J>
+static inline J msm_plane(const G1Jac* planes, size_t i) {
+  return jac_load(planes[i], (const J*)nullptr);
+}
+
+template <class J>
+static inline J msm_set_value_t(const J* planes, uint32_t cols) {
+  J v = planes[6];
+  for (int t = 5; t >= 0; t--) v = jac_add(jac_dbl(v), planes[t]);
+  if (cols == 128) {
+    for (int t = 6; t >= 0; t--) v = jac_add(jac_dbl(v), planes[7 + t]);
+    return jac_add(v, planes[14]);
+  }
+  J u = planes[13];
+  for (int t = 5; t >= 0; t--) u = jac_add(jac_dbl(u), planes[7 + t]);
+  for (uint32_t l = cols; l > 1; l >>= 1) v = jac_dbl(v);
+  return jac_add(jac_add(v, u), planes[14]);
+}
+template <class J>
+static inline J msm_set_value_of_t(const G1Jac* planes, uint32_t cols) {
+  J pl[MSM_SET_POINTS];
+  for (uint32_t q = 0; q < MSM_SET_POINTS; q++) pl[q] = msm_plane<J>(planes, q);
+  return msm_set_value_t(pl, cols);
+}
+
+template <class J>
+static inline J msm_fold_sets_t(const G1Jac* pairs, uint32_t Wb, uint32_t M, uint32_t cols) {
+  if (Wb == 1) return msm_set_value_of_t<J>(pairs, cols);
+  J planes[MSM_SET_POINTS];
+  for (uint32_t q = 0; q < MSM_SET_POINTS; q++) {
+    planes[q] = msm_plane<J>(pairs, q);
+    for (uint32_t s = 1; s < Wb; s++) planes[q] = jac_add(planes[q], msm_plane<J>(pairs, (size_t)MSM_SET_POINTS * s + q));
+  }
+  J acc = msm_set_value_t(planes, cols);
+  J run = J::identity(), weighted = J::identity();
+  for (uint32_t s = Wb - 1; s >= 1; s--) {
+    run = jac_add(run, msm_plane<J>(pairs, (size_t)MSM_SET_POINTS * s + MSM_SET_POINTS - 1));
+    weighted = jac_add(weighted, run);
+  }
+  for (uint32_t l = M; l > 1; l >>= 1) weighted = jac_dbl(weighted);
+  return jac_add(acc, weighted);
+}
+
+template <class J>
+static inline J msm_fold_window_range_t(const G1Jac* pairs, uint32_t w_lo, uint32_t w_hi, uint32_t c, uint32_t cols) {
+  J acc = J::identity();
+  if (c >= 2 && cols == (1u << (c - 1))) {
+    for (int w = (int)w_hi - 1; w >= (int)w_lo; w--) {
+      const G1Jac* pl = pairs + (size_t)MSM_SET_POINTS * w;
+      acc = jac_dbl(acc);
+      for (int t = (int)c - 2; t >= 0; t--) acc = jac_add(jac_dbl(acc), msm_plane<J>(pl, 7 + t));
+      acc = jac_add(acc, msm_plane<J>(pl, 14));
+    }
+    return acc;
+  }
+  for (int w = (int)w_hi - 1; w >= (int)w_lo; w--) {
+    for (uint32_t j = 0; j < c; j++) acc = jac_dbl(acc);
+    acc = jac_add(acc, msm_set_value_of_t<J>(pairs + (size_t)MSM_SET_POINTS * w, cols));
+  }
+  return acc;
+}
+template <class J>
+static inline J msm_fold_windows_t(const G1Jac* pairs, uint32_t W, uint32_t c, uint32_t cols) {
+  return msm_fold_window_range_t<J>(pairs, 0, W, c, cols);
+}
+
+static inline uint32_t msm_fold_split_at(uint32_t W) { return W / 2; }
+template <class J>
+static inline J msm_fold_join_t(const J& high, const J& low, uint32_t W, uint32_t c) {
+  J acc = high;
+  for (uint32_t j = 0; j < c * msm_fold_split_at(W); j++) acc = jac_dbl(acc);
+  return jac_add(acc, low);
+}
+template <class J>
+static inline J msm_fold_windows_split_t(const G1Jac* pairs, uint32_t W, uint32_t c, uint32_t cols) {
+  const uint32_t mid = msm_fold_split_at(W);
+  const J high = msm_fold_window_range_t<J>(pairs, mid, W, c, cols), low = msm_fold_window_range_t<J>(pairs, 0, mid, c, cols);
+  return msm_fold_join_t(high, low, W, c);
+}
+
+}
diff --git a/sha2_on_cq_halo2_amd/csrc/msm_multi.hip b/sha2_on_cq_halo2_amd/csrc/msm_multi.hip
--- a/sha2_on_cq_halo2_amd/csrc/msm_multi.hip
+++ b/sha2_on_cq_halo2_amd/csrc/msm_multi.hip
@@ -1,4 +1,5 @@
 #include <algorithm>
+#include <atomic>
 #include <cstdlib>
 #include <cstring>
 #include <vector>
@@ -108,16 +109,29 @@
   return CQ_OK;
 }
 
-int msm_multi_end(cq_ctx* c, MsmPending& pend, uint64_t* out_jac) {
+int msm_multi_end(cq_ctx* c, MsmPending& pend, uint64_t* out_jac, bool split_long) {
   if (int wrc = c->wait(c->stream, "msm: waiting for the launch")) return wrc;
-  struct Item { const MsmPending::Launch* ln; uint32_t j; };
+  struct Item { const MsmPending::Launch* ln; uint32_t j; int half; size_t split; };
+  struct Split { HJac part[2]; std::atomic<int> done{0}; };
   std::vector<Item> items;
-  size_t sets = 0;
+  size_t sets = 0, nsplit = 0, msms = 0, long_chains = 0;
+  for (auto& ln : pend.launches) {
+    msms += ln.batch;
+    if (!ln.empty) sets += (size_t)ln.batch * ln.L->Wb;
+    if (ln.short_path && ln.L->W >= 2) long_chains += ln.batch;
+  }
+  const bool use_pool = sets > 6;
+  const bool split = split_long && use_pool && long_chains && msms + long_chains <= c->pool().workers() + 1;
   for (auto& ln : pend.launches)
     for (uint32_t j = 0; j < ln.batch; j++) {
-      items.push_back({&ln, j});
-      if (!ln.empty) sets += ln.L->Wb;
-    }
+      if (split && ln.short_path && ln.L->W >= 2) {
+        items.push_back({&ln, j, 1, nsplit});
+        items.push_back({&ln, j, 0, nsplit++});
+      } else {
+        items.push_back({&ln, j, -1, 0});
+      }
+    }
+  std::vector<Split> splits(nsplit);
   const G1Jac* host = (const G1Jac*)pend.host;
   auto fold = [&](size_t i) {
     const MsmPending::Launch& ln = *items[i].ln;
@@ -129,13 +143,20 @@
     }
     const G1Jac* res = host + ln.slot;
     const MsmLayout& L = *ln.L;
-    G1Jac r = L.pre ? msm_fold_sets(res + (size_t)MSM_SET_POINTS * j * L.Wb, L.Wb, L.M, L.cols)
-                    : msm_fold_windows(res + (size_t)MSM_SET_POINTS * j * L.W, L.W, L.c, L.cols);
-    r.x.to_limbs64(o);
-    r.y.to_limbs64(o + 4);
-    r.z.to_limbs64(o + 8);
+    if (items[i].half >= 0) {
+      const G1Jac* sums = res + (size_t)MSM_SET_POINTS * j * L.W;
+      const uint32_t mid = msm_fold_split_at(L.W);
+      Split& sp = splits[items[i].split];
+      sp.part[items[i].half] = items[i].half ? msm_fold_window_range_t<HJac>(sums, mid, L.W, L.c, L.cols)
+                                             : msm_fold_window_range_t<HJac>(sums, 0, mid, L.c, L.cols);
+      if (sp.done.fetch_add(1) == 1) msm_fold_join_t(sp.part[1], sp.part[0], L.W, L.c).to_limbs64(o);
+      return;
+    }
+    const HJac r = L.pre ? msm_fold_sets_t<HJac>(res + (size_t)MSM_SET_POINTS * j * L.Wb, L.Wb, L.M, L.cols)
+                         : msm_fold_windows_t<HJac>(res + (size_t)MSM_SET_POINTS * j * L.W, L.W, L.c, L.cols);
+    r.to_limbs64(o);
   };
-  if (sets > 6) {
+  if (use_pool) {
     c->pool().parallel_for(items.size(), fold);
   } else {
     for (size_t i = 0; i < items.size(); i++) fold(i);
diff --git a/sha2_on_cq_halo2_amd/csrc/prover_lookup.hip b/sha2_on_cq_halo2_amd/csrc/prover_lookup.hip
--- a/sha2_on_cq_halo2_amd/csrc/prover_lookup.hip
+++ b/sha2_on_cq_halo2_amd/csrc/prover_lookup.hip
@@ -136,7 +136,7 @@
     for (size_t l = 0; l < PL; l++)
       for (int which = 2; which <= 3; which++) { sc.push_back(plk_buf(l, which)); bs.push_back(pk->params->g_lagrange); ln.push_back(n); }
     std::vector<int> f_linear(L, 0);
-    std::vector<G1Jac> f_host(L);
+    std::vector<HJac> f_host(L);
     for (size_t l = 0; l < L; l++) {
       f_linear[l] = 1;
       for (int64_t pj : pk->lookups[l].prog) f_linear[l] &= pj < 0;
@@ -163,8 +163,8 @@
     f_job.t = c->pool().submit(f_lin.size(), [&](size_t i) {
       const size_t l = f_lin[i];
       const auto& lcols = pk->lookups[l].cols;
-      G1Jac acc = jac_from_affine(advice_commitments[lcols[0]]);
-      for (size_t j = 1; j < lcols.size(); j++) acc = jac_add(host_scalar_mul(acc, theta), jac_from_affine(advice_commitments[lcols[j]]));
+      HJac acc = HJac::from_affine(advice_commitments[lcols[0]]);
+      for (size_t j = 1; j < lcols.size(); j++) acc = jac_add_mixed(host_scalar_mul(acc, theta), HAffine::from(advice_commitments[lcols[j]]));
       f_host[l] = acc;
     });
     {
@@ -190,7 +190,7 @@
     for (size_t q = 0; q < 2 * PL; q++)
       if (!tr.write_point(cm[q])) return c->fail(CQ_ERR_TRANSCRIPT, "permuted lookup commitment is the identity");
     for (size_t l = 0; l < L; l++) {
-      const G1Affine f_cm = f_linear[l] ? jac_to_affine(f_host[l]) : cm[f_slot[l]];
+      const G1Affine f_cm = f_linear[l] ? jac_to_affine(f_host[l]).to() : cm[f_slot[l]];
       if (!tr.write_point(f_cm)) return c->fail(CQ_ERR_TRANSCRIPT, "f commitment is the identity");
       if (!tr.write_point(early_m ? m_commitments[l] : cm[m_first + l])) return c->fail(CQ_ERR_TRANSCRIPT, "m commitment is the identity");
     }
diff --git a/sha2_on_cq_halo2_amd/csrc/prover_support.hip b/sha2_on_cq_halo2_amd/csrc/prover_support.hip
--- a/sha2_on_cq_halo2_amd/csrc/prover_support.hip
+++ b/sha2_on_cq_halo2_amd/csrc/prover_support.hip
@@ -5,10 +5,10 @@
 
 namespace {
 
-void batch_normalize(const std::vector<G1Jac>& in, std::vector<G1Affine>& out) {
+void batch_normalize(const std::vector<HJac>& in, std::vector<G1Affine>& out) {
   out.resize(in.size());
-  std::vector<Fq> pref(in.size());
-  Fq acc = Fq::one();
+  std::vector<HFq> pref(in.size());
+  HFq acc = HFq::one();
   for (size_t i = 0; i < in.size(); i++) {
     pref[i] = acc;
     if (!in[i].is_identity()) acc = acc * in[i].z;
@@ -19,15 +19,11 @@
       out[i] = G1Affine::identity();
       continue;
     }
-    Fq zi = pref[i] * acc;
+    HFq zi = pref[i] * acc;
     acc = acc * in[i].z;
-    Fq zi2 = zi.sqr();
-    out[i] = {in[i].x * zi2, in[i].y * zi2 * zi};
-  }
-}
-
-G1Jac jac_from_limbs(const uint64_t* l) {
-  return {Fq::from_limbs64(l), Fq::from_limbs64(l + 4), Fq::from_limbs64(l + 8)};
+    HFq zi2 = zi.sqr();
+    out[i] = HAffine{in[i].x * zi2, in[i].y * zi2 * zi}.to();
+  }
 }
 
 }
@@ -78,7 +74,7 @@
   const auto t0 = std::chrono::steady_clock::now();
   if (trace_host) hipStreamSynchronize(c->stream);
   const auto t1 = std::chrono::steady_clock::now();
-  int rc = msm_multi_end(c, pend, jac.data());
+  int rc = msm_multi_end(c, pend, jac.data(), true);
   if (rc != CQ_OK) return rc;
   const auto t2 = std::chrono::steady_clock::now();
   struct Report {
@@ -89,18 +85,18 @@
                       std::chrono::duration<double, std::micro>(std::chrono::steady_clock::now() - c_).count());
     }
   } report{trace_host, t0, t1, t2};
-  std::vector<G1Jac> j(count);
+  std::vector<HJac> j(count);
   if (pk->sharded()) {
     std::vector<uint64_t> all((size_t)pk->shard_world * count * 12);
     int arc = shard_allgather_host(pk, jac.data(), all.data(), count * 12 * sizeof(uint64_t));
     if (arc != CQ_OK) return arc;
     for (size_t i = 0; i < count; i++) {
-      G1Jac acc = G1Jac::identity();
-      for (uint32_t r = 0; r < pk->shard_world; r++) acc = jac_add(acc, jac_from_limbs(all.data() + ((size_t)r * count + i) * 12));
+      HJac acc = HJac::identity();
+      for (uint32_t r = 0; r < pk->shard_world; r++) acc = jac_add(acc, HJac::from_limbs64(all.data() + ((size_t)r * count + i) * 12));
       j[i] = acc;
     }
   } else {
-    for (size_t i = 0; i < count; i++) j[i] = jac_from_limbs(jac.data() + 12 * i);
+    for (size_t i = 0; i < count; i++) j[i] = HJac::from_limbs64(jac.data() + 12 * i);
   }
   batch_normalize(j, out);
   return CQ_OK;
```
